# alipbcs/ZetaRay

Hardware: NVIDIA H100
Metric: Mpaths/s (1spp ReSTIR PT, 1080p) (higher is better)
Workload: dtype f32

## Files before the change

zetaray_b200/csrc/rpt.cu:

```cuda
#include "zr_rpt_io.cuh"
#include "zr_rpt_spatial.h"
#include "zr_schedule.h"

namespace zr
{
namespace
{
    using namespace RPT;

    __device__ __align__(8) float c_disk512[1024];

#ifndef ZR_PT_THREADS
#define ZR_PT_THREADS 768
#endif
    struct PtParked
    {
        Reservoir r;
        Reconnection rc;
        uint32_t pad;
    };
    static_assert(sizeof(PtParked) % 4 == 0 && (sizeof(PtParked) / 4) % 2 == 1, "PtParked must be an odd number of words");
    constexpr size_t PT_SMEM_BYTES = (size_t)ZR_PT_THREADS * sizeof(PtParked);

    template<uint32_t MF>
    __global__ void ZR_LB(ZR_PT_THREADS) k_pathtrace(SceneDev sc, FrameView f, RptParams prm, zr_rpt_reservoir* __restrict__ res,
        float4* __restrict__ target, float4* __restrict__ finalImg, uint32_t dispX, uint32_t dispY, const uint32_t* __restrict__ order)
    {
        using SD = BSDF::ShadingDataT<MF>;
        extern __shared__ PtParked s_ptParked[];
        const zr_frame_constants& fc = f.fc;
        const long long t0 = clock64();
        uint2 sg = make_uint2(0, 0);
        const uint32_t groupFlat = order[blockIdx.x] * (ZR_PT_THREADS / 128) + (threadIdx.x >> 7);
        const uint32_t tInGroup = threadIdx.x & 127;
        uint2 px = make_uint2(0xffffffffu, 0xffffffffu);
        if (groupFlat < dispX * dispY)
            px = SwizzleThreadGroup(groupFlat, 0, tInGroup & 15, tInGroup >> 4, 16, 8, dispX, 16, 4, 16 * dispY, sg);
        bool inBounds = px.x < f.W && px.y < f.H && px.y >= prm.rowBegin && px.y < prm.rowEnd;
        const size_t idx = (size_t)px.y * f.W + px.x;
        bool alive = false;
        if (inBounds)
        {
            const GFlags flags = FlagsAt(f.core, f.W, px.x, px.y);
            if (flags.invalid || flags.emissive)
            {
                if (!fc.Accumulate || !fc.CameraStatic)
                    finalImg[idx] = f4(0, 0, 0, 0);
                inBounds = false;
            }
        }
        float3 pos = f3(0), normal = f3(0), li = f3(0), throughput = f3(0), throughput_k = f3(1), tr = f3(1);
        SD surface;
        BSDF::BSDFSample bsdfSample = BSDF::BSDFSample::Init();
        HitEmissive nextHit;
        nextHit.hit = false;
        Reconnection& rc = s_ptParked[threadIdx.x].rc;
        Reservoir& r = s_ptParked[threadIdx.x].r;
        rc = Reconnection::Init();
        r = Reservoir::Init();
        PrevHit prevHit;
        prevHit.alpha_lobe = 0; prevHit.wi = f3(0); prevHit.pdf = 0; prevHit.lobe = BSDF::DIFFUSE_R;
        float eta_curr = BSDF::ETA_AIR, eta_next = BSDF::DEFAULT_ETA_MAT;
        bool inTranslucentMedium = false;
        int bounce = 0, maxNumBounces = 0;
        RNG rngReplay, rngThread, rngGroup;
        rngReplay.State = rngThread.State = rngGroup.State = 0;
        uint32_t sampleSetIdx = 0;
        uint32_t seedReplay0 = 0;

        if (inBounds)
        {
            const PixelT<SD> p = LoadPixel<SD>(f, sc, f.core, f.coat, px.x, px.y, false, px.x, px.y);
            rngGroup = RNG::Init4(sg.x, sg.y, fc.FrameNum, 1);
            const uint3 state = RNG::PCG3d(make_uint3(px.x, px.y, fc.FrameNum));
            rngReplay = RNG::InitSeed(state.x);
            rngThread = RNG::InitSeed(state.y);
            seedReplay0 = state.x;
            maxNumBounces = (int)(p.surface.specTr ? prm.maxGlossyTrBounces : prm.maxNonTrBounces);
            bsdfSample = BSDF::SampleBSDF(p.normal, p.surface, rngReplay);
            if (dot(bsdfSample.bsdfOverPdf, bsdfSample.bsdfOverPdf) != 0)
            {
                sampleSetIdx = rngGroup.UniformUintBounded_Faster(sc.numSampleSets);
                pos = p.pos; normal = p.normal; surface = p.surface;
                throughput = bsdfSample.bsdfOverPdf;
                prevHit.alpha_lobe = BSDF::LobeAlpha(p.surface, bsdfSample.lobe);
                prevHit.lobe = bsdfSample.lobe; prevHit.wi = bsdfSample.wi; prevHit.pdf = bsdfSample.pdf;
                eta_curr = dot(p.normal, bsdfSample.wi) < 0 ? p.eta_next : BSDF::ETA_AIR;
                inTranslucentMedium = eta_curr != BSDF::ETA_AIR;
                alive = true;
            }
        }
        ZR_PHASE();
        if (alive)
            nextHit = FindClosestEmissive(sc, pos, normal, bsdfSample.wi, surface.Transmissive());

        while (__syncthreads_or(alive))
        {
            bool atRR = false;
            Hit hitInfo;
            float prevBsdfSamplePdf = 0; BSDF::LOBE prevBsdfSampleLobe = BSDF::DIFFUSE_R;
            const int pathVertex = bounce + 2;
            if (alive && !nextHit.hit)
                alive = false;
            if (alive)
            {
                hitInfo = HitAttributes(sc, nextHit.geoIdx, nextHit.primIdx, nextHit.bary, nextHit.t);
                const float3 newPos = mad(hitInfo.t, bsdfSample.wi, pos);
                if (!GetMaterialData(sc, -bsdfSample.wi, eta_curr, hitInfo, surface, eta_next))
                    alive = false;
                else
                {
                    pos = newPos;
                    normal = hitInfo.normal;
                    prevBsdfSamplePdf = bsdfSample.pdf;
                    prevBsdfSampleLobe = bsdfSample.lobe;
                    tr = f3(1);
                    if (inTranslucentMedium && surface.TrDepthGt0())
                    {
                        const float3 c = surface.baseColor_Fr0_TrCol;
                        const float3 extCoeff = f3(-zr_logf(c.x), -zr_logf(c.y), -zr_logf(c.z)) / surface.trDepth;
                        tr = f3(zr_expf(-hitInfo.t * extCoeff.x), zr_expf(-hitInfo.t * extCoeff.y), zr_expf(-hitInfo.t * extCoeff.z));
                        throughput *= tr;
                    }
                }
            }
            ZR_PHASE();
            BSDF::BSDFSample nextBsdfSample = bsdfSample;
            const int nextBounce = pathVertex - 1;
            if (alive && nextBounce <= maxNumBounces)
                nextBsdfSample = BSDF::SampleBSDF(hitInfo.normal, surface, rngReplay);
            ZR_PHASE();
            RaySetup rs; rs.go = false;
            RayHit rh; rh.hit = false;
            if (alive)
            {
                rs = SetupClosestEmissive(pos, hitInfo.normal, nextBsdfSample.wi, surface.Transmissive());
                if (rs.go)
                    rh = TraceClosest(sc, rs.o, nextBsdfSample.wi, rs.tmin, FLT_MAX_);
            }
            ZR_PHASE();
            NeeLightState nee;
            nee.facing = false; nee.ld = f3(0);
            bool lightSample = false;
            uint32_t seed_nee = 0;
            if (alive)
            {
                nextHit = FinishClosestEmissive(sc, rs, rh, nextBsdfSample.wi);
                const DirectLightingEstimate ls_b = NEE_Bsdf_Finish(sc, pos, surface, nextBounce, maxNumBounces, nextBsdfSample, nextHit);
                if (nextHit.HitWasEmissive())
                {
                    const float3 fOverPdf = throughput * ls_b.ld;
                    li += fOverPdf;
                    rc.L = Reconnection::half3(ls_b.ld * throughput_k);
                    MaybeSetCase2OrCase3(pathVertex, pos, hitInfo.normal, hitInfo.t, hitInfo.ID, hitInfo.meshIdx, surface,
                        prevHit, ls_b, 0, rc, prm.alpha_min);
                    r.Update(Math::Luminance(fOverPdf), fOverPdf, rc, rngThread);
                }
                lightSample = !IsSpecularSurface(surface);
                if (lightSample)
                {
                    seed_nee = rngThread.State;
                    SD surfNee = surface;
                    nee = NEE_Emissive_Begin(sc, pos, hitInfo.normal, surfNee, sampleSetIdx, rngThread);
                }
            }
            ZR_PHASE();
            if (lightSample && nee.facing && dot(nee.ld, nee.ld) > 0)
            {
                const RaySetup seg = SetupSegment(pos, nee.ret.wi, nee.t, hitInfo.normal, nee.ret.ID, surface.Transmissive());
                const bool visible = seg.go ? !TraceAnyExcept(sc, seg.o, nee.ret.wi, seg.tmin, seg.tmax, nee.ret.ID) : false;
                nee.ld *= visible ? 1.0f : 0.0f;
            }
            ZR_PHASE();
            if (lightSample)
            {
                float bsdfPdf = 0;
                if (nee.facing && dot(nee.ld, nee.ld) > 0)
                {
                    SD surfNee = surface;
                    surfNee.SetWi(nee.ret.wi, hitInfo.normal);
                    bsdfPdf = BSDF::BSDFSamplerPdf(hitInfo.normal, surfNee, nee.ret.wi, rngThread);
                    bsdfPdf *= nee.dwdA;
                }
                const DirectLightingEstimate ls = NEE_Emissive_Finish(nee, bsdfPdf);
                const float3 fOverPdf = throughput * ls.ld;
                li += fOverPdf;
                if (rc.IsCase2() || rc.IsCase3())
                    rc.Clear();
                rc.L = Reconnection::half3(ls.ld * throughput_k);
                MaybeSetCase2OrCase3(pathVertex, pos, hitInfo.normal, hitInfo.t, hitInfo.ID, hitInfo.meshIdx, surface,
                    prevHit, ls, seed_nee, rc, prm.alpha_min);
                r.Update(Math::Luminance(fOverPdf), fOverPdf, rc, rngThread);
            }
            if (alive)
            {
                bsdfSample = nextBsdfSample;
                if (bounce >= (maxNumBounces - 1))
                    alive = false;
                else
                {
                    if (rc.IsCase2() || rc.IsCase3())
                        rc.Clear();
                    bounce++;
                    atRR = true;
                }
            }
            const uint32_t rrMask = __ballot_sync(0xffffffffu, atRR);
            if (rrMask == 0)
                continue;
            const int rrBounce = __shfl_sync(0xffffffffu, bounce, __ffs(rrMask) - 1);
            const bool doRR = prm.russianRoulette && (rrBounce >= 3);
            float waveThroughput = 0.0f;
            if (doRR)
                waveThroughput = WaveMax32(atRR ? Math::Luminance(throughput) : -FLT_MAX_);
            if (atRR)
            {
                do
                {
                    if (doRR && waveThroughput < 1)
                    {
                        const float p_terminate = fmaxf(0.05f, 1 - waveThroughput);
                        if (rngGroup.Uniform() < p_terminate) { alive = false; break; }
                        throughput /= (1 - p_terminate);
                        throughput_k /= ((int)rc.k <= bounce) ? (1 - p_terminate) : 1.0f;
                    }
                    if (dot(bsdfSample.bsdfOverPdf, bsdfSample.bsdfOverPdf) == 0) { alive = false; break; }
                    const float alpha_lobe = BSDF::LobeAlpha(surface, bsdfSample.lobe);
                    if (rc.Empty() && CanReconnect(prevHit.alpha_lobe, alpha_lobe, prevHit.lobe, bsdfSample.lobe, prm.alpha_min))
                    {
                        rc.SetCase1(pathVertex, pos, hitInfo.t, hitInfo.normal, hitInfo.ID, hitInfo.meshIdx, -surface.wo,
                            prevBsdfSampleLobe, prevBsdfSamplePdf, bsdfSample.wi, bsdfSample.lobe, bsdfSample.pdf);
                        throughput_k = f3(1);
                    }
                    if ((int)rc.k <= bounce)
                        throughput_k *= bsdfSample.bsdfOverPdf * tr;
                    const bool transmitted = dot(normal, bsdfSample.wi) < 0;
                    throughput *= bsdfSample.bsdfOverPdf;
                    eta_curr = transmitted ? (eta_curr == BSDF::ETA_AIR ? eta_next : BSDF::ETA_AIR) : eta_curr;
                    inTranslucentMedium = eta_curr != BSDF::ETA_AIR;
                    prevHit.alpha_lobe = alpha_lobe;
                    prevHit.lobe = bsdfSample.lobe;
                    prevHit.wi = bsdfSample.wi;
                    prevHit.pdf = bsdfSample.pdf;
                } while (false);
            }
        }

        AccountCost(prm.costMap, f.W, f.H, px.x, px.y, t0);
        if (!inBounds)
            return;
        r.rc.seed_replay = seedReplay0;
        const float targetLum = Math::Luminance(r.target);
        r.W = targetLum > 0 ? fmaxf(r.w_sum / targetLum, 1.0f) : 0;
        if (prm.temporalResample || prm.resetTemporal)
        {
            zr_rpt_reservoir rec;
            r.Write(rec, 0);
            StoreRecord(&res[idx], rec);
        }
        if (prm.temporalResample)
        {
            r.target = Math::Sanitize(r.target);
            target[idx] = f4(r.target.x, r.target.y, r.target.z, 0.0f);
        }
        else
        {
            li = isnan3(li) ? f3(0) : li;
            if (fc.Accumulate && fc.CameraStatic)
            {
                const float4 prev = finalImg[idx];
                finalImg[idx] = f4(prev.x + li.x, prev.y + li.y, prev.z + li.z, prev.w);
            }
            else
                finalImg[idx] = f4(li.x, li.y, li.z, 0.0f);
        }
    }

    __global__ void __launch_bounds__(256) k_spatial_search(FrameView f, RptParams prm, uint16_t* __restrict__ neighbor)
    {
        const zr_frame_constants& fc = f.fc;
        const uint32_t x = blockIdx.x * 32 + (threadIdx.x & 31);
        const uint32_t y = prm.rowBegin + blockIdx.y * 8 + (threadIdx.x >> 5);
        if (x >= f.W || y >= f.H || y >= prm.rowEnd) return;
        const size_t idx = (size_t)y * f.W + x;
        const uint4 c = ld128(&f.core[idx]);
        const GFlags flags = DecodeFlags(c.w & 0xff);
        if (flags.invalid || flags.emissive) return;
        const float roughness = (float)((c.w >> 8) & 0xff) / 255.0f;
        const float viewDepth = asfloat(c.x);
        const float2 renderDimF = f2((float)f.W, (float)f.H);
        const float2 jitter = f2(fc.CurrCameraJitter[0], fc.CurrCameraJitter[1]);
        const float3 pos = Math::WorldPosFromScreenSpace(f2((float)x, (float)y), renderDimF, viewDepth, fc.TanHalfFOV,
            fc.AspectRatio, fc.CurrViewInv, jitter);
        const float3 normal = Math::DecodeUnitVector(Math::DecodeUNorm2(c.y));
        const uint3 h = RNG::PCG3d(make_uint3(x, y, fc.FrameNum));
        RNG rng = RNG::Init(h.x, h.y, fc.FrameNum);
        const float u0 = rng.Uniform();
        const uint32_t offset = rng.UniformUint();
        const float theta = u0 * TWO_PI;
        float sinTheta, cosTheta;
        zr_sincosf(theta, &sinTheta, &cosTheta);
        int foundX = 0xffff, foundY = 0xffff;
        int sxs[3], sys[3];
        bool inside[3];
        uint4 cand[3];
#pragma unroll
        for (uint32_t i = 0; i < 3; i++)
        {
            const uint32_t si = (offset + i) & 511;
            const float2 sampleUV = __ldg(reinterpret_cast<const float2*>(c_disk512) + si);
            float2 rotated = f2(dot(sampleUV, f2(cosTheta, -sinTheta)), dot(sampleUV, f2(sinTheta, cosTheta)));
            rotated = rotated * 15.0f;
            sxs[i] = (int)rintf((float)x + rotated.x); sys[i] = (int)rintf((float)y + rotated.y);
            inside[i] = !(sxs[i] < 0 || sys[i] < 0 || sxs[i] >= (int)f.W || sys[i] >= (int)f.H) && !(sxs[i] == (int)x && sys[i] == (int)y);
            cand[i] = inside[i] ? ld128(&f.core[(size_t)sys[i] * f.W + sxs[i]]) : make_uint4(0, 0, 0, 0);
        }
#pragma unroll
        for (uint32_t i = 0; i < 3; i++)
        {
            if (foundX != 0xffff || !inside[i]) continue;
            const int sxp = sxs[i], syp = sys[i];
            const uint4 sc4 = cand[i];
            const GFlags sf = DecodeFlags(sc4.w & 0xff);
            if (sf.invalid || sf.emissive) continue;
            if (flags.metallic != sf.metallic) continue;
            if (flags.transmissive != sf.transmissive) continue;
            const float sampleRoughness = (float)((sc4.w >> 8) & 0xff) / 255.0f;
            if (fabsf(sampleRoughness - roughness) > 0.05f) continue;
            const float3 samplePos = Math::WorldPosFromScreenSpace(f2((float)sxp, (float)syp), renderDimF, asfloat(sc4.x),
                fc.TanHalfFOV, fc.AspectRatio, fc.CurrViewInv, jitter);
            const float3 sampleNormal = Math::DecodeUnitVector(Math::DecodeUNorm2(sc4.y));
            if (!(fabsf(dot(normal, samplePos - pos)) <= 0.01f * viewDepth)) continue;
            if (dot(sampleNormal, normal) < 0.9f) continue;
            foundX = sxp; foundY = syp;
        }
        uint32_t mx, my;
        if (foundX == 0xffff) { mx = 0xff; my = 0xff; }
        else { mx = (uint32_t)(foundX - (int)x + 32); my = (uint32_t)(foundY - (int)y + 32); }
        neighbor[idx] = (uint16_t)((mx & 0xff) | ((my & 0xff) << 8));
    }

    __global__ void __launch_bounds__(256) k_sort(FrameView f, int mode, uint32_t spatialFlag, const zr_rpt_reservoir* __restrict__ resCurr,
        const zr_rpt_reservoir* __restrict__ resPrev, const uint16_t* __restrict__ neighbor, uint16_t* __restrict__ threadMap,
        uint32_t dispX, uint32_t dispY, uint32_t tileRow0)
    {
        enum { SUCCESS = 0, INVALID_PIXEL = 1, NOT_FOUND = 2, EMPTY = 4 };
        __shared__ unsigned long long s_warp[8];
        const uint32_t Gx = blockIdx.x, Gy = blockIdx.y + tileRow0, Gidx = threadIdx.x;
        const uint32_t GTx = Gidx & 15, GTy = Gidx >> 4;
        const bool againstEdge = (Gx == dispX - 1) || (Gy == dispY - 1);
        const bool lastGroup = (Gx == dispX - 1) && (Gy == dispY - 1);
        int dxs[4], dys[4], cls[4];
        uint32_t result[4];
#pragma unroll
        for (int i = 0; i < 4; i++)
        {
            const int gtx = (int)GTx * 2 + (i & 1), gty = (int)GTy * 2 + (i >> 1);
            const int dx = (int)(Gx * 32) + gtx, dy = (int)(Gy * 32) + gty;
            dxs[i] = dx; dys[i] = dy;
            int nx = 0, ny = 0;
            uint32_t err = SUCCESS;
            if ((uint32_t)dx >= f.W || (uint32_t)dy >= f.H)
                err = INVALID_PIXEL;
            else
            {
                const GFlags flags = FlagsAt(f.core, f.W, dx, dy);
                if (flags.invalid || flags.emissive)
                    err = INVALID_PIXEL;
                else if (mode == 1)
                {
                    if (!PrevPixel(f, dx, dy, nx, ny)) err = NOT_FOUND;
                }
                else if (mode == 3)
                {
                    if (!NeighborOf(f, neighbor, dx, dy, nx, ny)) err = NOT_FOUND;
                }
            }
            bool skip = err != SUCCESS;
            uint32_t k = Reconnection::EMPTY;
            if (err == SUCCESS)
            {
                const zr_rpt_reservoir* src = (mode == 1) ? resPrev : resCurr;
                const int sx = (mode == 1 || mode == 3) ? nx : dx, sy = (mode == 1 || mode == 3) ? ny : dy;
                const uint32_t kk = __ldg(&src[(size_t)sy * f.W + sx].meta) & 0xf;
                k = kk == Reconnection::EMPTY ? kk : kk + 2;
            }
            uint32_t res = err;
            if (k == Reconnection::EMPTY) { res |= EMPTY; skip = true; }
            bool edge = false;
            if (skip && againstEdge && ((uint32_t)dx < f.W) && ((uint32_t)dy < f.H))
            {
                res = SUCCESS; skip = false; edge = true;
            }
            int c = 4;
            if (!skip)
            {
                if (k == 2) c = 0;
                else if (k == 3) c = 1;
                else if (k == 4) c = 2;
                else c = 3;
                (void)edge;
            }
            cls[i] = c;
            result[i] = res;
        }
        auto writeOutput = [&](int dx, int dy, int mgx, int mgy, uint32_t res)
        {
            if ((Gx == dispX - 1) && (Gy != dispY - 1)) { const int t = mgx; mgx = mgy; mgy = t; }
            const int mx = (int)(Gx * 32) + mgx, my = (int)(Gy * 32) + mgy;
            uint32_t error;
            if (mode == 1) error = res & (spatialFlag ? (INVALID_PIXEL | NOT_FOUND) : INVALID_PIXEL);
            else if (mode == 3) error = res & INVALID_PIXEL;
            else error = res & (INVALID_PIXEL | EMPTY);
            if ((uint32_t)mx < f.W && (uint32_t)my < f.H)
            {
                const uint32_t ux = (uint32_t)(dx - mx + 31), uy = (uint32_t)(dy - my + 31);
                threadMap[(size_t)my * f.W + mx] = (uint16_t)(ux | (uy << 7) | ((error > 0 ? 1u : 0u) << 15));
            }
        };
        if (lastGroup)
        {
#pragma unroll
            for (int i = 0; i < 4; i++)
                writeOutput(dxs[i], dys[i], (int)GTx * 2 + (i & 1), (int)GTy * 2 + (i >> 1), result[i]);
            return;
        }
        unsigned long long mine = 0;
#pragma unroll
        for (int i = 0; i < 4; i++) mine += 1ull << (11 * cls[i]);
        unsigned long long incl = mine;
        const uint32_t lane = Gidx & 31, warp = Gidx >> 5;
#pragma unroll
        for (int off = 1; off < 32; off <<= 1)
        {
            const unsigned long long n = __shfl_up_sync(0xffffffffu, incl, off);
            if (lane >= (uint32_t)off) incl += n;
        }
        if (lane == 31) s_warp[warp] = incl;
        __syncthreads();
        unsigned long long warpOff = 0, total = 0;
        for (uint32_t w = 0; w < 8; w++)
        {
            const unsigned long long v = s_warp[w];
            if (w < warp) warpOff += v;
            total += v;
        }
        const unsigned long long excl = warpOff + incl - mine;
        uint32_t base[5];
        uint32_t acc = 0;
#pragma unroll
        for (int c = 0; c < 5; c++) { base[c] = acc; acc += (uint32_t)((total >> (11 * c)) & 0x7ff); }
        uint32_t within[5] = { 0, 0, 0, 0, 0 };
#pragma unroll
        for (int i = 0; i < 4; i++)
        {
            const int c = cls[i];
            const uint32_t rank = base[c] + (uint32_t)((excl >> (11 * c)) & 0x7ff) + within[c];
            within[c]++;
            writeOutput(dxs[i], dys[i], (int)(rank & 31), (int)(rank >> 5), result[i]);
        }
    }
}
}

struct zr_indirect_pass
{
    uint32_t width = 0, height = 0;
    struct Sized
    {
        zr::Planes planes{ "zr_indirect_pass" };
        zr_rpt_reservoir* d_res[2] = { nullptr, nullptr };
        float4* d_target = nullptr;
        float4* d_final = nullptr;
        uint16_t* d_neighbor = nullptr;
        uint16_t* d_threadMap = nullptr;
        zr::SpatialQueued queued;
    } sz;
    zr::ShiftStreams shiftStreams;
    int currTemporalIdx = 0;
    bool isTemporalReservoirValid = false;
    bool resetTemporalTextures = true;
    bool patternLoaded = false;
    zr::LightingStrip strip{ "zr_indirect_pass" };
    zr_indirect_params params = Defaults();

    static zr_indirect_params Defaults()
    {
        zr_indirect_params p{};
        p.max_non_tr_bounces = 3; p.max_glossy_tr_bounces = 4; p.russian_roulette = 1; p.temporal_resample = 1;
        p.num_spatial_passes = 1; p.M_max_temporal = 10; p.M_max_spatial = 8; p.boiling_suppression = 1;
        p.sort_temporal = 1; p.sort_spatial = 1; p.alpha_min = 0.175f * 0.175f;
        return p;
    }

    zr_status Setup()
    {
        decltype(&zr::k_pathtrace<zr::BSDF::MF_ALL>) const kernels[2] = { zr::k_pathtrace<zr::BSDF::MF_NONE>, zr::k_pathtrace<zr::BSDF::MF_ALL> };
        for (const auto kernel : kernels)
            ZR_TRY(zr::ReserveParkedSmem(kernel, ZR_PT_THREADS, zr::PT_SMEM_BYTES, "zr_indirect_pass: k_pathtrace"));
        return shiftStreams.Init();
    }

    zr_status OnWindowResized(uint32_t w, uint32_t h)
    {
        const size_t n = (size_t)w * h;
        Sized next;
        for (int i = 0; i < 2; i++) ZR_TRY(next.planes.Alloc(next.d_res[i], n));
        ZR_TRY(next.planes.Alloc(next.d_threadMap, n));
        ZR_TRY(next.planes.Alloc(next.d_target, n));
        ZR_TRY(next.planes.Alloc(next.d_final, n));
        ZR_TRY(next.planes.Alloc(next.d_neighbor, n));
        ZR_TRY(next.queued.Build(w, h, next.d_res[0], next.d_res[1]));
        ZR_TRY(next.planes.Clear());
        sz = std::move(next);
        width = w; height = h;
        strip.ForgetSize();
        ResetFlags();
        return ZR_OK;
    }

    void ResetFlags() { currTemporalIdx = 0; isTemporalReservoirValid = false; resetTemporalTextures = true; }
    zr_status ResetTemporal()
    {
        ZR_TRY(sz.planes.Clear());
        ResetFlags();
        return ZR_OK;
    }

    zr_status LoadPattern()
    {
        if (patternLoaded) return ZR_OK;
        float pat[1024];
        zr_status st = zr::read_asset("zr_indirect_pass", "disk512.bin", pat, sizeof(pat));
        if (st != ZR_OK) return st;
        ZR_CUDA(cudaMemcpyToSymbol(zr::c_disk512, pat, 4096));
        patternLoaded = true;
        return ZR_OK;
    }

    zr_status Render(const zr_frame_inputs* in, cudaStream_t stream)
    {
        using namespace zr;
        FrameView f;
        zr_status st = LightingFrame("zr_indirect_pass", in, width, height, f);
        if (st != ZR_OK) return st;
        st = LoadPattern();
        if (st != ZR_OK) return st;

        const bool doTemporal = params.temporal_resample && isTemporalReservoirValid;
        const bool doSpatial = (params.num_spatial_passes > 0) && doTemporal;
        if (doTemporal && (!in->prev.d_core || !in->prev.d_coat))
        {
            set_error("zr_indirect_pass_render: temporal reuse needs the previous G-buffer");
            return ZR_ERR_INVALID_ARG;
        }
        RptParams prm;
        prm.maxNonTrBounces = params.max_non_tr_bounces; prm.maxGlossyTrBounces = params.max_glossy_tr_bounces;
        prm.russianRoulette = params.russian_roulette; prm.M_max_temporal = params.M_max_temporal; prm.M_max_spatial = params.M_max_spatial;
        prm.boilingSuppression = params.boiling_suppression; prm.sortSpatial = params.sort_spatial; prm.alpha_min = params.alpha_min;
        prm.temporalResample = doTemporal; prm.resetTemporal = resetTemporalTextures; prm.spatialFlag = doSpatial;
        prm.rowBegin = strip.rowBegin; prm.rowEnd = strip.ClampedRowEnd(height);
        prm.costMap = strip.d_costMap;
        st = strip.Schedule(width, height, 16, 8, ZR_PT_THREADS / 128);
        if (st != ZR_OK) return st;
        const uint32_t rows = prm.rowEnd - prm.rowBegin;

        int cur = currTemporalIdx;
        const uint32_t dispX = (width + 15) / 16, dispY = (height + 7) / 8;
        const bool plain = (in->scene->materialFeatures & BSDF::MF_ALL) == 0;
        ZR_PROF("k_pathtrace", stream);
        (plain ? k_pathtrace<BSDF::MF_NONE> : k_pathtrace<BSDF::MF_ALL>)<<<strip.sched[0].count, ZR_PT_THREADS, PT_SMEM_BYTES, stream>>>(in->scene->dev, f, prm, sz.d_res[cur], sz.d_target, sz.d_final, dispX, dispY,
            strip.sched[0].d_order);
        ZR_LAUNCH_CHECK();
        if (doTemporal)
        {
            st = sz.queued.RunTemporal(shiftStreams, in->scene->dev, f, prm, sz.d_res[cur], sz.d_res[1 - cur], sz.d_target, sz.d_final, plain, stream);
            if (st != ZR_OK) return st;
        }
        strip.Exchange(sz.d_res[cur], width, height, 64u, stream);
        if (doSpatial)
        {
            for (uint32_t pass = 0; pass < params.num_spatial_passes; pass++)
            {
                ZR_PROF("k_spatial_search", stream);
                k_spatial_search<<<dim3((width + 31) / 32, (rows + 7) / 8), 256, 0, stream>>>(f, prm, sz.d_neighbor);
                ZR_LAUNCH_CHECK();
                zr_rpt_reservoir* rin = sz.d_res[cur];
                zr_rpt_reservoir* rout = sz.d_res[1 - cur];
                cur = 1 - cur;
                if (params.sort_spatial)
                {
                    const uint32_t sx = (width + 31) / 32, sy = (height + 31) / 32;
                    ZR_PROF("k_sort", stream);
                    const uint32_t ty0 = prm.rowBegin / 32, ty1 = (prm.rowEnd + 31) / 32;
                    k_sort<<<dim3(sx, ty1 - ty0), 256, 0, stream>>>(f, 3, 1u, rin, nullptr, sz.d_neighbor, sz.d_threadMap, sx, sy, ty0);
                    ZR_LAUNCH_CHECK();
                }
                st = sz.queued.Run(shiftStreams, in->scene->dev, f, prm, rin, rout, sz.d_target, sz.d_final, sz.d_neighbor, sz.d_threadMap, plain, stream);
                if (st != ZR_OK) return st;
                strip.Exchange(rout, width, height, 64u, stream);
            }
        }
        isTemporalReservoirValid = true;
        currTemporalIdx = 1 - cur;
        resetTemporalTextures = false;
        return ZR_OK;
    }
};

extern "C"
{
    zr_status zr_indirect_pass_create(uint32_t width, uint32_t height, zr_indirect_pass** out) { return zr::CreatePass("zr_indirect_pass", width, height, out); }
    zr_status zr_indirect_pass_resize(zr_indirect_pass* p, uint32_t width, uint32_t height) { return zr::ResizePass("zr_indirect_pass", p, width, height); }
    zr_status zr_indirect_pass_reset_temporal(zr_indirect_pass* p) { return zr::ResetPass(p); }
    zr_status zr_indirect_pass_default_params(zr_indirect_params* out) { return zr::DefaultParams<zr_indirect_pass>(out); }
    zr_status zr_indirect_pass_set_params(zr_indirect_pass* p, const zr_indirect_params* params)
    {
        if (!p || !params) return ZR_ERR_INVALID_ARG;
        if (params->max_non_tr_bounces < 1 || params->max_non_tr_bounces > 8 || params->max_glossy_tr_bounces < 1 ||
            params->max_glossy_tr_bounces > 8 || params->M_max_temporal > 15 || params->M_max_spatial > 15 || params->num_spatial_passes > 2)
        {
            zr::set_error("zr_indirect_pass_set_params: value out of range (bounces 1..8, M_max <= 15, spatial passes <= 2)");
            return ZR_ERR_INVALID_ARG;
        }
        p->params = *params;
        return ZR_OK;
    }
    zr_status zr_indirect_pass_render(zr_indirect_pass* p, const zr_frame_inputs* in, void* stream)
    {
        if (!p) return ZR_ERR_INVALID_ARG;
        return p->Render(in, (cudaStream_t)stream);
    }
    zr_status zr_indirect_pass_get_output(zr_indirect_pass* p, zr_indirect_output id, zr_image2d* out)
    {
        if (!p || !out) return ZR_ERR_INVALID_ARG;
        const uint32_t w = p->width, h = p->height;
        switch (id)
        {
        case ZR_INDIRECT_FINAL: *out = zr_image2d{ p->sz.d_final, w, h, w * 16u, 16u }; break;
        case ZR_INDIRECT_RESERVOIR_CURR: *out = zr_image2d{ p->sz.d_res[1 - p->currTemporalIdx], w, h, w * 64u, 64u }; break;
        case ZR_INDIRECT_RESERVOIR_PREV: *out = zr_image2d{ p->sz.d_res[p->currTemporalIdx], w, h, w * 64u, 64u }; break;
        case ZR_INDIRECT_TARGET: *out = zr_image2d{ p->sz.d_target, w, h, w * 16u, 16u }; break;
        case ZR_INDIRECT_NEIGHBOR: *out = zr_image2d{ p->sz.d_neighbor, w, h, w * 2u, 2u }; break;
        case ZR_INDIRECT_THREADMAP_NTC: *out = zr_image2d{ p->sz.d_threadMap, w, h, w * 2u, 2u }; break;
        default: zr::set_error("zr_indirect_pass_get_output: unknown output id"); return ZR_ERR_INVALID_ARG;
        }
        return ZR_OK;
    }
    zr_status zr_indirect_pass_describe_io(zr_indirect_pass* p, zr_resource_use* uses, int* n)
    {
        if (!p || !uses || !n) return ZR_ERR_INVALID_ARG;
        uses[0] = zr_resource_use{ ZR_RES_GBUFFER_CURR, 0 };
        uses[1] = zr_resource_use{ ZR_RES_GBUFFER_PREV, 0 };
        uses[2] = zr_resource_use{ ZR_RES_SCENE_BVH, 0 };
        uses[3] = zr_resource_use{ ZR_RES_ALIAS_TABLE, 0 };
        uses[4] = zr_resource_use{ ZR_RES_INDIRECT_FINAL, 1 };
        *n = 5;
        return ZR_OK;
    }
    zr_status zr_indirect_pass_set_halo_exchange(zr_indirect_pass* p, zr_halo_exchange_fn fn, void* user) { return p ? p->strip.SetHaloExchange(fn, user) : ZR_ERR_INVALID_ARG; }
    zr_status zr_indirect_pass_set_schedule_costs(zr_indirect_pass* p, const double* h_tile_cost, uint32_t tiles_x, uint32_t tiles_y)
    {
        return p ? p->strip.SetScheduleCosts(h_tile_cost, tiles_x, tiles_y, p->width, p->height) : ZR_ERR_INVALID_ARG;
    }
    zr_status zr_indirect_pass_set_cost_map(zr_indirect_pass* p, void* d_cycles) { return p ? p->strip.SetCostMap(d_cycles) : ZR_ERR_INVALID_ARG; }
    zr_status zr_indirect_pass_set_rows(zr_indirect_pass* p, uint32_t y0, uint32_t y1) { return p ? p->strip.SetRows(y0, y1, p->height) : ZR_ERR_INVALID_ARG; }
    void zr_indirect_pass_destroy(zr_indirect_pass* p) { delete p; }
}
```

zetaray_b200/csrc/rpt_spatial.cu:

```cuda
#include "zr_rpt_spatial.h"
#include "zr_rpt_shift.cuh"
#include "zr_tma.cuh"

namespace zr
{
namespace
{
    using namespace RPT;

    __global__ void __launch_bounds__(256) k_spatial_classify(FrameView f, RptParams prm, const zr_rpt_reservoir* __restrict__ resIn,
        const uint16_t* __restrict__ neighbor, uint32_t* __restrict__ queue, uint32_t* __restrict__ counters, uint32_t capacity)
    {
        __shared__ uint32_t s_count[SpatialQueued::NUM_CLASSES], s_base[SpatialQueued::NUM_CLASSES];
        const uint32_t x = blockIdx.x * 32 + (threadIdx.x & 31);
        const uint32_t y = prm.rowBegin + blockIdx.y * 8 + (threadIdx.x >> 5);
        if (threadIdx.x < SpatialQueued::NUM_CLASSES) s_count[threadIdx.x] = 0;
        __syncthreads();
        uint32_t cls[2] = { NO_ITEM, NO_ITEM };
        if (x < f.W && y < f.H && y < prm.rowEnd)
        {
            const GFlags flags = FlagsAt(f.core, f.W, (int)x, (int)y);
            int nx = 0, ny = 0;
            if (!(flags.invalid || flags.emissive) && NeighborOf(f, neighbor, (int)x, (int)y, nx, ny))
            {
                const uint4 q0 = ld128(&resIn[(size_t)y * f.W + x]);
                const uint4 qn = ld128(&resIn[(size_t)ny * f.W + nx]);
                const bool selfEmpty = (q0.x & 0xf) == Reconnection::EMPTY, nEmpty = (qn.x & 0xf) == Reconnection::EMPTY;
                const uint32_t M_n = (qn.x >> 4) & 0xf;
                if (asfloat(q0.y) != 0 && !selfEmpty && M_n > 0) cls[0] = ShiftClass(q0.x);
                if (!nEmpty) cls[1] = ShiftClass(qn.x);
            }
        }
        const uint32_t item[2] = { x | (y << 16), x | (y << 16) | (1u << 31) };
        AppendItems(cls, item, queue, counters, capacity, s_count, s_base);
    }

    struct MergeSmem
    {
        uint4 rec[2][1024][4];
        float val[2][1024];
        float sum[2][1024];
        uint8_t cls[1024];
        uint8_t visited[1024];
        unsigned long long bar[2];
    };

    __global__ void __launch_bounds__(1024, 1) k_spatial_merge(const CUtensorMap* __restrict__ pMapIn, FrameView f, RptParams prm,
        const zr_rpt_reservoir* __restrict__ resIn, zr_rpt_reservoir* __restrict__ resOut, const float4* __restrict__ target,
        float4* __restrict__ finalImg, const uint16_t* __restrict__ neighbor, const uint16_t* __restrict__ threadMap,
        const ShiftResult* __restrict__ shiftRes, uint32_t tilesX, uint32_t tileRow0, uint32_t numTiles, uint32_t swizzled)
    {
        extern __shared__ __align__(1024) unsigned char smemRaw[];
        MergeSmem& sm = *reinterpret_cast<MergeSmem*>(smemRaw);
        const zr_frame_constants& fc = f.fc;
        const uint32_t t = threadIdx.x, lane = t & 31, warp = t >> 5;
        constexpr uint32_t TILE_BYTES = 1024 * 64;

        if (t == 0)
        {
            tma::MbarInit(reinterpret_cast<uint64_t*>(&sm.bar[0]), 1);
            tma::MbarInit(reinterpret_cast<uint64_t*>(&sm.bar[1]), 1);
            tma::FenceBarrierInit();
        }
        __syncthreads();
        auto issue = [&](uint32_t tile, uint32_t stage)
        {
            const uint32_t tx = tile % tilesX, ty = tileRow0 + tile / tilesX;
            uint64_t* bar = reinterpret_cast<uint64_t*>(&sm.bar[stage]);
            tma::MbarArriveExpectTx(bar, TILE_BYTES);
            if (swizzled) tma::Load3D(&sm.rec[stage][0][0], pMapIn, bar, 0, (int32_t)(tx * 16), (int32_t)(ty * 32));
            else tma::Load2D(&sm.rec[stage][0][0], pMapIn, bar, (int32_t)(tx * 32 * 8), (int32_t)(ty * 32));
        };
        if (t == 0 && blockIdx.x < numTiles)
            issue(blockIdx.x, 0);

        uint32_t pfFlags = 0xff, pfNb = 0xffff, pfMap = 0x8000;
        float4 pfTg = f4(0, 0, 0, 0);
        auto prefetch = [&](uint32_t tile)
        {
            const uint32_t tX = tile % tilesX, tY = tileRow0 + tile / tilesX;
            const uint32_t px = tX * 32 + lane, py = tY * 32 + warp;
            pfFlags = 0xff; pfNb = 0xffff; pfMap = 0x8000;
            if (px < f.W && py < f.H && py >= prm.rowBegin && py < prm.rowEnd)
            {
                const size_t i = (size_t)py * f.W + px;
                pfFlags = __ldg(&f.core[i].w) & 0xff;
                pfNb = __ldg(&neighbor[i]);
                pfTg = __ldg(&target[i]);
            }
            const uint32_t sx = tX * 32 + (warp & 3) * 8 + (lane & 7), sy = tY * 32 + (warp >> 2) * 4 + (lane >> 3);
            if (sx < f.W && sy < f.H)
                pfMap = prm.sortSpatial ? __ldg(&threadMap[(size_t)sy * f.W + sx]) : (31u | (31u << 7));
        };
        if (blockIdx.x < numTiles)
            prefetch(blockIdx.x);

        uint32_t it = 0;
        for (uint32_t tile = blockIdx.x; tile < numTiles; tile += gridDim.x, it++)
        {
            const uint32_t stage = it & 1, parity = (it >> 1) & 1;
            const uint32_t tileX = tile % tilesX, tileY = tileRow0 + tile / tilesX;
            if (t == 0 && tile + gridDim.x < numTiles)
            {
                tma::FenceProxyAsync();
                issue(tile + gridDim.x, stage ^ 1);
            }
            const int x = (int)(tileX * 32 + lane), y = (int)(tileY * 32 + warp);
            const bool inImage = (uint32_t)x < f.W && (uint32_t)y < f.H;
            const size_t idx = inImage ? (size_t)y * f.W + x : 0;
            bool act = false;
            {
                const GFlags flags = DecodeFlags(pfFlags);
                act = !(flags.invalid || flags.emissive);
            }
            int nx = 0, ny = 0;
            bool hasN = false;
            const float4 tg = pfTg;
            const uint32_t mapEnc = pfMap;
            uint4 sh0 = make_uint4(0, 0, 0, 0);
            float2 sh1 = f2(0, 0);
            uint4 n0 = make_uint4(Reconnection::EMPTY, 0, 0, 0), n1 = make_uint4(0, 0, 0, 0);
            if (act)
            {
                const uint32_t ox = pfNb & 0xff, oy = pfNb >> 8;
                hasN = ox != 0xff;
                nx = (int)ox - 32 + x; ny = (int)oy - 32 + y;
                if (hasN)
                {
                    const uint4* nrec = reinterpret_cast<const uint4*>(&resIn[(size_t)ny * f.W + nx]);
                    n0 = __ldg(&nrec[0]); n1 = __ldg(&nrec[1]);
                    asm volatile("prefetch.global.L1 [%0];" :: "l"(nrec + 2));
                    const uint4* sp = reinterpret_cast<const uint4*>(&shiftRes[idx]);
                    sh0 = __ldg(&sp[0]);
                    sh1 = __ldg(reinterpret_cast<const float2*>(&sp[1]));
                }
            }
            if (tile + gridDim.x < numTiles)
                prefetch(tile + gridDim.x);
            sm.visited[t] = 0;
            tma::MbarWait(reinterpret_cast<uint64_t*>(&sm.bar[stage]), parity);

            zr_rpt_reservoir rec;
            {
                const uint4* line = &sm.rec[stage][t & ~1u][0];
                const uint32_t c0 = (t & 1u) * 4u, sw = swizzled ? ((t >> 1) & 7u) : 0u;
                uint4 v[4] = { line[(c0 + 0) ^ sw], line[(c0 + 1) ^ sw], line[(c0 + 2) ^ sw], line[(c0 + 3) ^ sw] };
                memcpy(&rec, v, 64);
            }
            Reservoir r_curr = Reservoir::Load_NonReconnection(rec);
            r_curr.target = f3(tg.x, tg.y, tg.z);
            const float wsum0 = act ? r_curr.w_sum : 0.0f;
            uint32_t M_max = prm.M_max_spatial;
            M_max = !r_curr.rc.Empty() && r_curr.rc.lobe_k_min_1 == BSDF::GLOSSY_T ? (M_max < 4 ? M_max : 4) : M_max;
            uint32_t cls = 0, M_new = 0;
            bool changed = false, surfKMin1Tr = false;
            zr_rpt_reservoir recN;
            Reservoir r_spatial = Reservoir::Init();
            if (act && !hasN)
                cls = 1;
            else if (act)
            {
                memset(&recN, 0, sizeof(recN));
                memcpy(&recN, &n0, 16); memcpy(reinterpret_cast<unsigned char*>(&recN) + 16, &n1, 16);
                r_spatial = Reservoir::Load_NonReconnection(recN);
                if ((r_curr.w_sum != 0) && !r_curr.rc.Empty() && (r_spatial.M > 0))
                {
                    const float target_spatial = sh1.x;
                    if (target_spatial > 0)
                    {
                        const float selfJ = (r_curr.rc.IsCase3() && r_curr.rc.lobe_k_min_1 == BSDF::ALL) ? 1.0f : asfloat(rec.jacobian_or_seed_nee);
                        const float targetLum_curr = r_curr.W > 0 ? r_curr.w_sum / r_curr.W : 0;
                        const float jacobian = selfJ > 0 ? sh1.y / selfJ : 0;
                        const float numerator = (float)r_curr.M * targetLum_curr;
                        const float denom = numerator + (float)r_spatial.M * target_spatial * jacobian;
                        const float m_curr = denom > 0 ? numerator / denom : 0;
                        r_curr.w_sum *= m_curr;
                    }
                }
                M_new = r_curr.M + r_spatial.M;
                if (r_spatial.rc.Empty())
                    cls = 2;
                else
                {
                    cls = 3;
                    M_max = r_spatial.rc.x_k_in_motion ? (M_max < 4 ? M_max : 4) : M_max;
                    r_spatial.rc.x_k_in_motion = false;
                    const float nJ = (r_spatial.rc.IsCase3() && r_spatial.rc.lobe_k_min_1 == BSDF::ALL) ? 1.0f : asfloat(recN.jacobian_or_seed_nee);
                    const float3 shTarget = f3(asfloat(sh0.x), asfloat(sh0.y), asfloat(sh0.z));
                    const float shJ = fabsf(asfloat(sh0.w));
                    surfKMin1Tr = (sh0.w >> 31) != 0;
                    const float targetLum_curr = Math::Luminance(shTarget);
                    const float targetLum_spatial = r_spatial.W > 0 ? r_spatial.w_sum / r_spatial.W : 0;
                    const float jacobian = nJ > 0 ? shJ / nJ : 0;
                    if (targetLum_curr > 1e-6f && jacobian > 1e-5f && jacobian < 100)
                    {
                        const uint3 h = RNG::PCG3d(make_uint3((uint32_t)x, (uint32_t)y, (uint32_t)y));
                        RNG rng = RNG::Init(h.x, h.z, fc.FrameNum + 511);
                        const float numerator = (float)r_spatial.M * targetLum_spatial;
                        const float denom = numerator / jacobian + (float)r_curr.M * targetLum_curr;
                        const float m_spatial = denom > 0 ? numerator / denom : 0;
                        const float w_spatial = m_spatial * r_spatial.W * targetLum_curr;
                        if (r_curr.Update(w_spatial, shTarget, r_spatial.rc, rng))
                        {
                            const uint4* nrec = reinterpret_cast<const uint4*>(&resIn[(size_t)ny * f.W + nx]);
                            const uint4 n2 = __ldg(&nrec[2]), n3 = __ldg(&nrec[3]);
                            memcpy(reinterpret_cast<unsigned char*>(&recN) + 32, &n2, 16);
                            memcpy(reinterpret_cast<unsigned char*>(&recN) + 48, &n3, 16);
                            r_spatial.Load_Reconnection(recN);
                            r_curr.rc = r_spatial.rc;
                            r_curr.rc.partialJacobian = shJ;
                            changed = true;
                        }
                    }
                    const float targetLum = Math::Luminance(r_curr.target);
                    r_curr.W = targetLum > 0 ? r_curr.w_sum / targetLum : 0;
                    r_curr.M = M_new;
                }
            }
            sm.val[0][t] = wsum0;
            sm.val[1][t] = act ? r_curr.w_sum : 0.0f;
            sm.cls[t] = (uint8_t)cls;
            __syncthreads();

            {
                const int sx = (int)(tileX * 32 + (warp & 3) * 8 + (lane & 7)), sy = (int)(tileY * 32 + (warp >> 2) * 4 + (lane >> 3));
                bool on = (uint32_t)sx < f.W && (uint32_t)sy < f.H;
                int lx = sx - (int)(tileX * 32), ly = sy - (int)(tileY * 32);
                if (mapEnc & (1u << 15)) on = false;
                lx += (int)(mapEnc & 0x3f) - 31;
                ly += (int)((mapEnc >> 7) & 0x3f) - 31;
                if (on && ((uint32_t)lx >= 32u || (uint32_t)ly >= 32u)) on = false;
                const uint32_t lp = on ? (uint32_t)(ly * 32 + lx) : 0;
                const float v0 = on ? sm.val[0][lp] : 0.0f, v1 = on ? sm.val[1][lp] : 0.0f;
                const uint32_t c = on ? sm.cls[lp] : 0;
                const float waveSum = WaveSum32(v0);
                float waveAcc = WaveSum32(c == 1 ? v1 : 0.0f);
                waveAcc += WaveSum32(c == 2 ? v1 : 0.0f);
                const float total = waveAcc + WaveSum32(c == 3 ? v1 : 0.0f);
                if (on)
                {
                    sm.sum[0][lp] = waveSum; sm.sum[1][lp] = total;
                    sm.visited[lp] = 1;
                }
            }
            __syncthreads();

            if (act && sm.visited[t])
            {
                const float avgEx0 = (sm.sum[0][t] - wsum0) / 32.0f;
                if (cls == 1)
                {
                    if (prm.boilingSuppression) SuppressOutlier(avgEx0, r_curr);
                    WriteOutputColor(fc, finalImg, idx, r_curr.target * r_curr.W);
                    CopyToNextFrame(rec, &resOut[idx], r_curr, M_max);
                }
                else if (cls == 2)
                {
                    if (prm.boilingSuppression) SuppressOutlier(avgEx0, r_curr);
                    const float targetLum = Math::Luminance(r_curr.target);
                    r_curr.W = targetLum > 0 ? r_curr.w_sum / targetLum : 0;
                    r_curr.M = M_new;
                    CopyToNextFrame(rec, &resOut[idx], r_curr, M_max);
                    WriteOutputColor(fc, finalImg, idx, r_curr.target * r_curr.W);
                }
                else
                {
                    if (prm.boilingSuppression)
                        SuppressOutlier((sm.sum[1][t] - r_curr.w_sum) / 32.0f, r_curr);
                    if (changed)
                    {
                        const uint32_t mmax = surfKMin1Tr ? (M_max < 4 ? M_max : 4) : M_max;
                        zr_rpt_reservoir out;
                        r_curr.Write(out, mmax);
                        StoreRecord(&resOut[idx], out);
                    }
                    else
                        CopyToNextFrame(rec, &resOut[idx], r_curr, M_max);
                    WriteOutputColor(fc, finalImg, idx, r_curr.target * r_curr.W);
                }
            }
            __syncthreads();
        }
    }
}

zr_status ShiftStreams::Init()
{
    int dev = 0;
    ZR_CUDA(cudaGetDevice(&dev));
    ZR_CUDA(cudaDeviceGetAttribute(&numSMs, cudaDevAttrMultiProcessorCount, dev));
    ZR_CUDA(cudaFuncSetAttribute(k_spatial_merge, cudaFuncAttributeMaxDynamicSharedMemorySize, (int)sizeof(MergeSmem)));
    ZR_TRY(SetupShifts<false>());
    ZR_TRY(SetupTemporalShifts());
    for (int i = 0; i < 2; i++)
    {
        ZR_CUDA(cudaStreamCreateWithFlags(&aux[i], cudaStreamNonBlocking));
        ZR_CUDA(cudaEventCreateWithFlags(&evJoin[i], cudaEventDisableTiming));
    }
    ZR_CUDA(cudaEventCreateWithFlags(&evFork, cudaEventDisableTiming));
    return ZR_OK;
}

ShiftStreams::~ShiftStreams()
{
    for (int i = 0; i < 2; i++)
    {
        if (aux[i]) cudaStreamDestroy(aux[i]);
        if (evJoin[i]) cudaEventDestroy(evJoin[i]);
    }
    if (evFork) cudaEventDestroy(evFork);
}

zr_status SpatialQueued::Build(uint32_t w, uint32_t h, const zr_rpt_reservoir* res0, const zr_rpt_reservoir* res1)
{
    width = w; height = h;
    const size_t n = (size_t)w * h;
    capacity = 2 * n;
    ZR_TRY(planes.Alloc(d_queue, NUM_CLASSES * capacity, false));
    ZR_TRY(planes.Alloc(d_counters, 16, false));
    ZR_TRY(planes.Alloc(d_shift, n));
    ZR_TRY(planes.Alloc(d_flags, n));
    ZR_TRY(planes.Alloc(d_maps, 2, false));
    const zr_rpt_reservoir* res[2] = { res0, res1 };
    CUtensorMap maps[2];
    swizzled = (w % 2) == 0;
    for (int i = 0; i < 2; i++)
    {
        mapBase[i] = res[i];
        bool ok;
        if (swizzled)
        {
            const uint64_t dims[3] = { 16, w / 2, h };
            const uint64_t strides[2] = { 128, (uint64_t)w * 64 };
            const uint32_t box[3] = { 16, 16, 32 };
            ok = tma::EncodeWords(&maps[i], res[i], 3, dims, strides, box, true);
        }
        else
            ok = tma::EncodePlane2D(&maps[i], res[i], w, h, 64, (uint64_t)w * 64, 32, 32);
        if (!ok)
        {
            set_error("zr_indirect_pass: cuTensorMapEncodeTiled failed for the %ux%u reservoir plane", w, h);
            return ZR_ERR_CUDA;
        }
    }
    ZR_CUDA(cudaMemcpy(d_maps, maps, sizeof(maps), cudaMemcpyHostToDevice));
    return planes.Clear();
}

zr_status SpatialQueued::Run(const ShiftStreams& ss, const SceneDev& sc, const FrameView& f, const RptParams& prm, const zr_rpt_reservoir* resIn,
    zr_rpt_reservoir* resOut, const float4* target, float4* finalImg, const uint16_t* neighbor, const uint16_t* threadMap, bool plain, cudaStream_t stream)
{
    const int plane = resIn == mapBase[0] ? 0 : (resIn == mapBase[1] ? 1 : -1);
    if (plane < 0) { set_error("zr_indirect_pass: spatial input is not one of the pass's reservoir planes"); return ZR_ERR_INVALID_ARG; }
    const uint32_t rows = prm.rowEnd - prm.rowBegin;
    ZR_CUDA(cudaMemsetAsync(d_counters, 0, 16 * sizeof(uint32_t), stream));
    {
        ZR_PROF("k_spatial_classify", stream);
        k_spatial_classify<<<dim3((width + 31) / 32, (rows + 7) / 8), 256, 0, stream>>>(f, prm, resIn, neighbor, d_queue, d_counters, (uint32_t)capacity);
        ZR_LAUNCH_CHECK();
    }
    {
        ZR_PROF("k_shift", stream);
        const zr_status ls = LaunchShifts<false>(*this, ss, sc, f, prm, resIn, nullptr, neighbor, plain, stream);
        zr::prof_after();
        if (ls != ZR_OK) return ls;
        cudaError_t e = cudaGetLastError();
        if (e != cudaSuccess) return zr::cuda_fail(e, "k_shift launch");
    }
    {
        const uint32_t tilesX = (width + 31) / 32;
        const uint32_t tileRow0 = prm.rowBegin / 32, tileRow1 = (prm.rowEnd + 31) / 32;
        const uint32_t numTiles = tilesX * (tileRow1 - tileRow0);
        const uint32_t grid = numTiles < (uint32_t)ss.numSMs ? numTiles : (uint32_t)ss.numSMs;
        ZR_PROF("k_spatial_merge", stream);
        k_spatial_merge<<<grid, 1024, sizeof(MergeSmem), stream>>>(d_maps + plane, f, prm, resIn, resOut, target, finalImg, neighbor, threadMap,
            d_shift, tilesX, tileRow0, numTiles, swizzled ? 1u : 0u);
        ZR_LAUNCH_CHECK();
    }
    return ZR_OK;
}
}
```

zetaray_b200/csrc/rpt_temporal.cu:

```cuda
#include "zr_rpt_spatial.h"
#include "zr_rpt_shift.cuh"

namespace zr
{
namespace
{
    using namespace RPT;
    enum : uint8_t { TF_OK = 1, TF_REPLAY_OK = 2 };

    __global__ void __launch_bounds__(256) k_temporal_classify(SceneDev sc, FrameView f, RptParams prm, const zr_rpt_reservoir* __restrict__ resCurr,
        const zr_rpt_reservoir* __restrict__ resPrev, uint8_t* __restrict__ tflags, uint32_t* __restrict__ queue, uint32_t* __restrict__ counters,
        uint32_t capacity)
    {
        __shared__ uint32_t s_count[SpatialQueued::NUM_CLASSES], s_base[SpatialQueued::NUM_CLASSES];
        const int x = (int)(blockIdx.x * 32 + (threadIdx.x & 31));
        const int y = (int)(prm.rowBegin + blockIdx.y * 8 + (threadIdx.x >> 5));
        if (threadIdx.x < SpatialQueued::NUM_CLASSES) s_count[threadIdx.x] = 0;
        __syncthreads();
        uint32_t cls[2] = { NO_ITEM, NO_ITEM };
        uint32_t flagBits = 0;
        if (x < (int)f.W && y < (int)f.H && y < (int)prm.rowEnd)
        {
            const size_t idx = (size_t)y * f.W + x;
            const GFlags flags = DecodeFlags(ld128(&f.core[idx]).w & 0xff);
            bool ok = !(flags.invalid || flags.emissive), okReplay = false;
            int ppx = 0, ppy = 0;
            if (ok)
            {
                ok = PrevPixel(f, x, y, ppx, ppy);
                if (ok)
                    ok = asfloat(__ldg(&f.pcore[(size_t)ppy * f.W + ppx].x)) != FLT_MAX_;
            }
            if (ok)
            {
                const Pixel cur = LoadPixel(f, sc, f.core, f.coat, x, y, false, x, y);
                const Pixel prev = LoadPixel(f, sc, f.pcore, f.pcoat, ppx, ppy, true, x, y);
                ok = PlaneHeuristic(prev.pos, cur.normal, cur.pos, cur.z, 1.0f);
                okReplay = ok && PlaneHeuristic(prev.pos, cur.normal, cur.pos, cur.z, 0.01f);
                const bool matOk = !(prev.flags.emissive || (fabsf(prev.roughness - cur.roughness) > 0.3f) ||
                    (prev.flags.transmissive != cur.flags.transmissive));
                ok = ok && matOk;
                okReplay = okReplay && matOk;
            }
            if (ok)
            {
                flagBits = TF_OK | (okReplay ? TF_REPLAY_OK : 0);
                const uint4 q0 = ld128(&resCurr[idx]);
                const uint4 qp = ld128(&resPrev[(size_t)ppy * f.W + ppx]);
                const bool selfEmpty = (q0.x & 0xf) == Reconnection::EMPTY, pEmpty = (qp.x & 0xf) == Reconnection::EMPTY;
                const uint32_t M_p = (qp.x >> 4) & 0xf;
                if (asfloat(q0.y) != 0 && M_p > 0 && !selfEmpty) cls[0] = ShiftClass(q0.x);
                if (!pEmpty) cls[1] = ShiftClass(qp.x);
            }
            tflags[idx] = (uint8_t)flagBits;
        }
        const uint32_t base = (uint32_t)x | ((uint32_t)y << 16) | ((flagBits & TF_REPLAY_OK) ? (1u << 30) : 0u);
        const uint32_t item[2] = { base, base | (1u << 31) };
        AppendItems(cls, item, queue, counters, capacity, s_count, s_base);
    }

    __global__ void __launch_bounds__(256, 4) k_temporal_merge(SceneDev sc, FrameView f, RptParams prm, zr_rpt_reservoir* __restrict__ resCurr,
        const zr_rpt_reservoir* __restrict__ resPrev, float4* __restrict__ target, float4* __restrict__ finalImg,
        const uint8_t* __restrict__ tflags, const ShiftResult* __restrict__ shiftRes)
    {
        const zr_frame_constants& fc = f.fc;
        const int x = (int)(blockIdx.x * 32 + (threadIdx.x & 31));
        const int y = (int)(prm.rowBegin + blockIdx.y * 8 + (threadIdx.x >> 5));
        if (x >= (int)f.W || y >= (int)f.H || y >= (int)prm.rowEnd) return;
        const size_t idx = (size_t)y * f.W + x;
        {
            const GFlags flags = DecodeFlags(ld128(&f.core[idx]).w & 0xff);
            if (flags.invalid || flags.emissive) return;
        }
        zr_rpt_reservoir rec;
        LoadRecord(&resCurr[idx], rec);
        Reservoir r_curr = Reservoir::Load_NonReconnection(rec);
        const float4 tg = target[idx];
        r_curr.target = f3(tg.x, tg.y, tg.z);
        const bool ok = (__ldg(&tflags[idx]) & TF_OK) != 0;
        if (!ok)
        {
            if (!prm.spatialFlag)
                WriteOutputColor(fc, finalImg, idx, r_curr.target * r_curr.W);
            return;
        }
        int ppx = 0, ppy = 0;
        PrevPixel(f, x, y, ppx, ppy);
        const size_t pidx = (size_t)ppy * f.W + ppx;
        zr_rpt_reservoir recPrev;
        LoadRecord(&resPrev[pidx], recPrev);
        Reservoir r_prev = Reservoir::Load_NonReconnection(recPrev);
        const uint4* sp = reinterpret_cast<const uint4*>(&shiftRes[idx]);

        if (r_curr.w_sum != 0 && r_prev.M > 0 && !r_curr.rc.Empty())
        {
            const float2 sh1 = __ldg(reinterpret_cast<const float2*>(&sp[1]));
            const float target_prev = sh1.x;
            if (target_prev > 0)
            {
                const float selfJ = (r_curr.rc.IsCase3() && r_curr.rc.lobe_k_min_1 == BSDF::ALL) ? 1.0f : asfloat(rec.jacobian_or_seed_nee);
                const float targetLum_curr = r_curr.W > 0 ? r_curr.w_sum / r_curr.W : 0;
                const float jacobian = selfJ > 0 ? sh1.y / selfJ : 0;
                const float m_curr = targetLum_curr / (targetLum_curr + (float)r_prev.M * target_prev * jacobian);
                r_curr.w_sum *= m_curr;
                rec.w_sum = r_curr.w_sum;
            }
        }

        const uint32_t M_new = r_curr.M + r_prev.M;
        const uint32_t M_max = prm.M_max_temporal;
        if (r_prev.rc.Empty())
        {
            const float targetLum = Math::Luminance(r_curr.target);
            r_curr.W = targetLum > 0 ? r_curr.w_sum / targetLum : 0;
            r_curr.M = M_new;
            const uint32_t k = r_curr.rc.Empty() ? r_curr.rc.k : (r_curr.rc.k > 2 ? r_curr.rc.k : 2) - 2;
            const uint32_t mm = r_curr.M < M_max ? r_curr.M : M_max;
            rec.meta = (rec.meta & 0xffffff00u) | ((k | (mm << 4)) & 0xff);
            rec.W = r_curr.W;
            st128(&resCurr[idx], make_uint4(rec.meta, asuint(rec.w_sum), asuint(rec.W), rec.L_b));
            if (!prm.spatialFlag)
                WriteOutputColor(fc, finalImg, idx, r_curr.target * r_curr.W);
            return;
        }
        r_prev.Load_Reconnection(recPrev);
        if (r_prev.rc.IsCase1() || r_prev.rc.IsCase2())
            XkToCurr(sc, r_prev.rc);
        const uint4 sh0 = __ldg(&sp[0]);
        const float3 shTarget = f3(asfloat(sh0.x), asfloat(sh0.y), asfloat(sh0.z));
        const float shJ = asfloat(sh0.w);
        const float targetLum_curr = Math::Luminance(shTarget);
        const float jacobian = r_prev.rc.partialJacobian > 0 ? shJ / r_prev.rc.partialJacobian : 0;
        bool changed = false;
        if (targetLum_curr > 1e-6f && jacobian > 1e-5f)
        {
            RNG rng = RNG::Init((uint32_t)y, (uint32_t)x, fc.FrameNum + 31);
            const float targetLum_prev = r_prev.W > 0 ? r_prev.w_sum / r_prev.W : 0;
            const float numerator = (float)r_prev.M * targetLum_prev;
            const float denom = numerator / jacobian + targetLum_curr;
            const float m_prev = denom > 0 ? numerator / denom : 0;
            const float w_prev = m_prev * r_prev.W * targetLum_curr;
            if (r_curr.Update(w_prev, shTarget, r_prev.rc, rng))
            {
                r_curr.rc.partialJacobian = shJ;
                changed = true;
            }
        }
        const float targetLum = Math::Luminance(r_curr.target);
        r_curr.W = targetLum > 0 ? r_curr.w_sum / targetLum : 0;
        r_curr.M = M_new;
        if (changed)
        {
            zr_rpt_reservoir out;
            r_curr.Write(out, M_max);
            StoreRecord(&resCurr[idx], out);
            if (prm.spatialFlag)
            {
                r_curr.target = Math::Sanitize(r_curr.target);
                target[idx] = f4(r_curr.target.x, r_curr.target.y, r_curr.target.z, 0.0f);
            }
        }
        else
        {
            r_curr.WriteReservoirData(rec, M_max);
            st128(&resCurr[idx], make_uint4(rec.meta, asuint(rec.w_sum), asuint(rec.W), rec.L_b));
        }
        if (!prm.spatialFlag)
            WriteOutputColor(fc, finalImg, idx, r_curr.target * r_curr.W);
    }
}

zr_status SetupTemporalShifts()
{
    return SetupShifts<true>();
}

zr_status SpatialQueued::RunTemporal(const ShiftStreams& ss, const SceneDev& sc, const FrameView& f, const RptParams& prm, zr_rpt_reservoir* resCurr,
    const zr_rpt_reservoir* resPrev, float4* target, float4* finalImg, bool plain, cudaStream_t stream)
{
    const uint32_t rows = prm.rowEnd - prm.rowBegin;
    const dim3 grid((width + 31) / 32, (rows + 7) / 8);
    ZR_CUDA(cudaMemsetAsync(d_counters, 0, 16 * sizeof(uint32_t), stream));
    {
        ZR_PROF("k_temporal_classify", stream);
        k_temporal_classify<<<grid, 256, 0, stream>>>(sc, f, prm, resCurr, resPrev, d_flags, d_queue, d_counters, (uint32_t)capacity);
        ZR_LAUNCH_CHECK();
    }
    {
        ZR_PROF("k_shift_temporal", stream);
        const zr_status ls = LaunchShifts<true>(*this, ss, sc, f, prm, resCurr, resPrev, nullptr, plain, stream);
        zr::prof_after();
        if (ls != ZR_OK) return ls;
        cudaError_t e = cudaGetLastError();
        if (e != cudaSuccess) return zr::cuda_fail(e, "k_shift (temporal) launch");
    }
    {
        ZR_PROF("k_temporal_merge", stream);
        k_temporal_merge<<<grid, 256, 0, stream>>>(sc, f, prm, resCurr, resPrev, target, finalImg, d_flags, d_shift);
        ZR_LAUNCH_CHECK();
    }
    return ZR_OK;
}
}
```

zetaray_b200/csrc/zr_rpt_io.cuh:

```cuda
#pragma once
#include "zr_rpt.cuh"
#include "zr_pixel.cuh"

namespace zr
{
struct RptParams
{
    uint32_t maxNonTrBounces, maxGlossyTrBounces, russianRoulette, M_max_temporal, M_max_spatial;
    uint32_t boilingSuppression, sortSpatial;
    float alpha_min;
    uint32_t temporalResample, resetTemporal, spatialFlag;
    uint32_t rowBegin, rowEnd;
    unsigned long long* costMap;
};

namespace
{
    using namespace RPT;

    ZR_D void LoadRecord(const zr_rpt_reservoir* __restrict__ p, zr_rpt_reservoir& r)
    {
        const uint4* q = reinterpret_cast<const uint4*>(p);
        uint4 v[4] = { q[0], q[1], q[2], q[3] };
        memcpy(&r, v, 64);
    }
    ZR_D void StoreRecord(zr_rpt_reservoir* __restrict__ p, const zr_rpt_reservoir& r)
    {
        uint4 v[4];
        memcpy(v, &r, 64);
        uint4* q = reinterpret_cast<uint4*>(p);
        q[0] = v[0]; q[1] = v[1]; q[2] = v[2]; q[3] = v[3];
    }
    ZR_D uint4 LoadQ0(const zr_rpt_reservoir* __restrict__ p) { return *reinterpret_cast<const uint4*>(p); }

    ZR_D bool NeighborOf(const FrameView& f, const uint16_t* __restrict__ neighbor, int x, int y, int& nx, int& ny)
    {
        const uint16_t nb = __ldg(&neighbor[(size_t)y * f.W + x]);
        const int ox = nb & 0xff, oy = nb >> 8;
        if (ox == 0xff) return false;
        nx = ox - 32 + x; ny = oy - 32 + y;
        return true;
    }

    ZR_D void SuppressOutlier(float waveAvgExclusive, Reservoir& r)
    {
        if (r.w_sum > 50 * waveAvgExclusive)
        {
            r.M = 0; r.w_sum = 0; r.W = 0; r.rc.Clear();
        }
    }

    ZR_D bool RecordSurvivesRoundTrip(const zr_rpt_reservoir& in)
    {
        const uint32_t wx = in.w_k & 0xffff, wy = in.w_k >> 16;
        const bool interior = wx != 0 && wx != 0xffff && wy != 0 && wy != 0xffff;
        const uint32_t r = in.L_rg & 0x7fff, g = (in.L_rg >> 16) & 0x7fff, b = in.L_b & 0x7fff;
        return interior && r <= 0x7c00 && g <= 0x7c00 && b <= 0x7c00;
    }

    ZR_D void CopyToNextFrame(const zr_rpt_reservoir& in, zr_rpt_reservoir* __restrict__ outPtr, Reservoir r_curr, uint32_t M_max)
    {
        if (!r_curr.rc.Empty() && RecordSurvivesRoundTrip(in))
        {
            zr_rpt_reservoir out = in;
            out.meta = r_curr.PackMeta(M_max);
            out.w_sum = Math::Sanitize(r_curr.w_sum);
            out.W = Math::Sanitize(r_curr.W);
            out.L_b = in.L_b & 0xffff;
            if (r_curr.rc.IsCase1()) { out.lightPdf = 0; out.dwdA = 0; out.seed_nee = 0; }
            else if (!r_curr.rc.IsCase2()) { out.dwdA = 0; out.seed_nee = 0; out.meshIdx = 0; }
            StoreRecord(outPtr, out);
        }
        else if (!r_curr.rc.Empty())
        {
            r_curr.Load_Reconnection(in);
            zr_rpt_reservoir out;
            r_curr.Write(out, M_max);
            StoreRecord(outPtr, out);
        }
        else
        {
            const uint4 old = LoadQ0(outPtr);
            const uint32_t k = r_curr.rc.k;
            const uint32_t mm = r_curr.M < M_max ? r_curr.M : M_max;
            st128(outPtr, make_uint4((old.x & 0xffffff00u) | ((k | (mm << 4)) & 0xff), asuint(r_curr.w_sum), asuint(r_curr.W), old.w));
        }
    }

    ZR_D bool PrevPixel(const FrameView& f, int x, int y, int& ppx, int& ppy)
    {
        const float2 renderDim = f2((float)f.W, (float)f.H);
        const float2 motionVec = unpack_snorm16x2(__ldg(&f.me[(size_t)y * f.W + x].x));
        const float2 currUV = f2((float)x + 0.5f, (float)y + 0.5f) / renderDim;
        const float2 prevUV = currUV - motionVec;
        const float2 pp = prevUV * renderDim;
        ppx = (int)pp.x; ppy = (int)pp.y;
        return !(prevUV.x < 0.0f || prevUV.y < 0.0f || prevUV.x > 1.0f || prevUV.y > 1.0f);
    }

    ZR_D bool PlaneHeuristic(float3 prevPos, float3 normal, float3 pos, float linearDepth, float th)
    {
        return fabsf(dot(normal, prevPos - pos)) <= th * linearDepth;
    }

    ZR_D void XkToPrev(const SceneDev& sc, Reconnection& rc)
    {
        const zr_mesh_instance md = LoadInstance(sc, rc.meshIdx);
        const float4 q_curr = normalize(Math::DecodeNormalized4(md.Rotation));
        const float3 T = f3(md.Translation[0], md.Translation[1], md.Translation[2]);
        const float3 x_local = Math::InverseTransformTRS(rc.x_k, T, q_curr, h3(md.Scale));
        const float3 prevTranslation = T - h3(md.dTranslation);
        const float4 q_prev = normalize(Math::DecodeNormalized4(md.PrevRotation));
        rc.x_k = Math::TransformTRS(x_local, prevTranslation, q_prev, h3(md.PrevScale));
    }
    ZR_D void XkToCurr(const SceneDev& sc, Reconnection& rc)
    {
        const zr_mesh_instance md = LoadInstance(sc, rc.meshIdx);
        const float3 T = f3(md.Translation[0], md.Translation[1], md.Translation[2]);
        const float3 dT = h3(md.dTranslation);
        const float3 prevTranslation = T - dT;
        const float4 q_prev = normalize(Math::DecodeNormalized4(md.PrevRotation));
        const float3 prevScale = h3(md.PrevScale), scale = h3(md.Scale);
        const float3 x_local = Math::InverseTransformTRS(rc.x_k, prevTranslation, q_prev, prevScale);
        const float4 q_curr = normalize(Math::DecodeNormalized4(md.Rotation));
        rc.x_k = Math::TransformTRS(x_local, T, q_curr, scale);
        const float4 dRot = f4(q_prev.x - q_curr.x, q_prev.y - q_curr.y, q_prev.z - q_curr.z, q_prev.w - q_curr.w);
        const float3 dScale = prevScale - scale;
        rc.x_k_in_motion = dot(dT, dT) > 0;
        rc.x_k_in_motion = rc.x_k_in_motion || dot(dRot, dRot) > 0;
        rc.x_k_in_motion = rc.x_k_in_motion || dot(dScale, dScale) > 0;
    }

    struct PrevHit { float alpha_lobe; float3 wi; float pdf; BSDF::LOBE lobe; };

    template<class SD>
    ZR_D void MaybeSetCase2OrCase3(int pathVertex, float3 pos, float3 normal, float t, uint32_t ID, uint32_t meshIdx,
        const SD& surface, const PrevHit& prevHit, const DirectLightingEstimate& ls, uint32_t seed_nee,
        Reconnection& rc, float alpha_min)
    {
        const float alpha_lobe_direct = BSDF::LobeAlpha(surface, ls.lobe);
        if (rc.Empty() && CanReconnect(prevHit.alpha_lobe, alpha_lobe_direct, prevHit.lobe, ls.lobe, alpha_min))
        {
            rc.SetCase2(pathVertex, pos, t, normal, ID, meshIdx, prevHit.wi, prevHit.lobe, prevHit.pdf, ls.wi, ls.lobe,
                ls.pdf_solidAngle, ls.lt, ls.pdf_light, ls.le, seed_nee, ls.dwdA);
        }
        if (rc.Empty() && (alpha_lobe_direct >= alpha_min))
        {
            rc.SetCase3(pathVertex + 1, ls.pos, ls.lt, ls.lobe, ls.ID, ls.le, ls.normal, ls.pdf_solidAngle, ls.pdf_light,
                ls.dwdA, ls.wi, ls.twoSided, seed_nee);
        }
    }

}
}
```

zetaray_b200/csrc/zr_rpt_shift.cuh:

```cuda
#pragma once
#include "zr_rpt_spatial.h"

namespace zr
{
namespace
{
    using namespace RPT;
#ifndef ZR_SHIFT_THREADS
#define ZR_SHIFT_THREADS 768
#endif
#ifndef ZR_SHIFT_MINBLOCKS
#define ZR_SHIFT_MINBLOCKS 1
#endif
    constexpr int SHIFT_THREADS = ZR_SHIFT_THREADS, SHIFT_MINBLOCKS = ZR_SHIFT_MINBLOCKS;
    constexpr uint32_t NO_ITEM = 0xffffffffu;

    struct ShiftParked
    {
        Reconnection rc;
        uint32_t pad;
    };
    static_assert(sizeof(ShiftParked) % 4 == 0 && (sizeof(ShiftParked) / 4) % 2 == 1, "ShiftParked must be an odd number of words");
    constexpr size_t SHIFT_SMEM_BYTES = (size_t)SHIFT_THREADS * sizeof(ShiftParked);

    ZR_D uint32_t ShiftClass(uint32_t meta)
    {
        const uint32_t kMin2 = meta & 0xf;
        const uint32_t lt_k = (meta >> 14) & 3, lt_k1 = (meta >> 16) & 3;
        const uint32_t c = lt_k1 != 0 ? 1u : (lt_k != 0 ? 2u : 0u);
        return c * 2 + (kMin2 > 0 ? 1u : 0u);
    }


    template<int CASE, bool REPLAY, bool TEMPORAL, uint32_t MF>
    __global__ void __launch_bounds__(SHIFT_THREADS, SHIFT_MINBLOCKS) k_shift(SceneDev sc, FrameView f, RptParams prm,
        const zr_rpt_reservoir* __restrict__ resIn, const zr_rpt_reservoir* __restrict__ resPrev, const uint16_t* __restrict__ neighbor,
        const uint32_t* __restrict__ queue, uint32_t* __restrict__ counters, uint32_t cls, ShiftResult* __restrict__ out)
    {
        using SD = BSDF::ShadingDataT<MF>;
        __shared__ uint32_t s_base;
        extern __shared__ ShiftParked s_shiftParked[];
        Reconnection& rc = s_shiftParked[threadIdx.x].rc;
        const uint32_t total = counters[cls];
        for (;;)
        {
            __syncthreads();
            if (threadIdx.x == 0) s_base = atomicAdd(&counters[8 + cls], (uint32_t)SHIFT_THREADS);
            __syncthreads();
            const uint32_t base = s_base;
            if (base >= total) break;
            const bool act = base + threadIdx.x < total;
            int x = 0, y = 0;
            uint32_t dir = 0;
            bool replayOk = act;
            PixelT<SD> p, pr;
            if (act)
            {
                const uint32_t item = __ldg(&queue[base + threadIdx.x]);
                x = (int)(item & 0xffff); y = (int)((item >> 16) & 0x3fff); dir = item >> 31;
                zr_rpt_reservoir rec;
                if (!TEMPORAL)
                {
                    int nx = 0, ny = 0;
                    NeighborOf(f, neighbor, x, y, nx, ny);
                    LoadRecord(dir == 0 ? &resIn[(size_t)y * f.W + x] : &resIn[(size_t)ny * f.W + nx], rec);
                    Reservoir r = Reservoir::Load_NonReconnection(rec);
                    r.rc.x_k_in_motion = false;
                    r.Load_Reconnection(rec);
                    rc = r.rc;
                    if (dir == 0) p = LoadPixel<SD>(f, sc, f.core, f.coat, nx, ny, false, x, y);
                    else p = LoadPixel<SD>(f, sc, f.core, f.coat, x, y, false, x, y);
                    if (REPLAY)
                    {
                        if (dir == 0) pr = LoadPixel<SD>(f, sc, f.core, f.coat, nx, ny, false, nx, ny);
                        else pr = p;
                    }
                }
                else
                {
                    replayOk = ((item >> 30) & 1) != 0;
                    int ppx = 0, ppy = 0;
                    PrevPixel(f, x, y, ppx, ppy);
                    LoadRecord(dir == 0 ? &resIn[(size_t)y * f.W + x] : &resPrev[(size_t)ppy * f.W + ppx], rec);
                    Reservoir r = Reservoir::Load_NonReconnection(rec);
                    r.Load_Reconnection(rec);
                    if (r.rc.IsCase1() || r.rc.IsCase2())
                    {
                        if (dir == 0) XkToPrev(sc, r.rc);
                        else XkToCurr(sc, r.rc);
                    }
                    rc = r.rc;
                    if (dir == 0) p = LoadPixel<SD>(f, sc, f.pcore, f.pcoat, ppx, ppy, true, x, y);
                    else p = LoadPixel<SD>(f, sc, f.core, f.coat, x, y, false, x, y);
                    if (REPLAY) pr = p;
                }
            }
            else
                rc = Reconnection::Init();
            OffsetPathContextT<SD> ctx = OffsetPathContextT<SD>::Init();
            if (REPLAY)
            {
                ZR_PHASE();
                ctx = Replay_kGt2_Sync(act && replayOk, sc, pr.pos, pr.normal, pr.eta_next, pr.surface, rc, prm.alpha_min);
                if (act && replayOk)
                    ctx = ctx.Quantize();
            }
            const OffsetPath shift = Shift2_Sync<CASE>(act, sc, p.pos, p.normal, p.eta_next, p.surface, rc, &ctx, prm.alpha_min);
            if (act)
            {
                ShiftResult* o = &out[(size_t)y * f.W + x];
                if (dir == 0)
                    *reinterpret_cast<float2*>(&o->ctsTargetLum) = f2(Math::Luminance(shift.target), shift.partialJacobian);
                else if (TEMPORAL)
                    st128(o, make_uint4(asuint(shift.target.x), asuint(shift.target.y), asuint(shift.target.z), asuint(shift.partialJacobian)));
                else
                {
                    const float J = shift.partialJacobian;
                    const float Jenc = J > 0 ? (shift.surfKMin1Tramsmissive ? -J : J) : 0.0f;
                    st128(o, make_uint4(asuint(shift.target.x), asuint(shift.target.y), asuint(shift.target.z), asuint(Jenc)));
                }
            }
        }
    }

    template<bool TEMPORAL>
    zr_status LaunchShifts(const SpatialQueued& q, const ShiftStreams& ss, const SceneDev& sc, const FrameView& f, const RptParams& prm,
        const zr_rpt_reservoir* resIn, const zr_rpt_reservoir* resPrev, const uint16_t* neighbor, bool plain, cudaStream_t stream)
    {
        const uint32_t grid = (uint32_t)ss.numSMs * SHIFT_MINBLOCKS;
        cudaStream_t s1 = ss.aux[0], s2 = ss.aux[1];
        ZR_CUDA(cudaEventRecord(ss.evFork, stream));
        ZR_CUDA(cudaStreamWaitEvent(s1, ss.evFork, 0));
        ZR_CUDA(cudaStreamWaitEvent(s2, ss.evFork, 0));
#define ZR_LAUNCH_SHIFT(CASE, REPLAY, CLS, STREAM) \
        (plain ? k_shift<CASE, REPLAY, TEMPORAL, BSDF::MF_NONE> : k_shift<CASE, REPLAY, TEMPORAL, BSDF::MF_ALL>)<<<grid, SHIFT_THREADS, SHIFT_SMEM_BYTES, STREAM>>>(sc, f, prm, resIn, resPrev, neighbor, q.d_queue + (size_t)(CLS) * q.capacity, \
            q.d_counters, CLS, q.d_shift); \
        zr::count_launch()
        ZR_LAUNCH_SHIFT(1, false, 0, stream);
        ZR_LAUNCH_SHIFT(2, false, 2, s1);
        ZR_LAUNCH_SHIFT(3, false, 4, s2);
        ZR_LAUNCH_SHIFT(1, true, 1, s1);
        ZR_LAUNCH_SHIFT(2, true, 3, s2);
        ZR_LAUNCH_SHIFT(3, true, 5, stream);
#undef ZR_LAUNCH_SHIFT
        ZR_CUDA(cudaEventRecord(ss.evJoin[0], s1));
        ZR_CUDA(cudaEventRecord(ss.evJoin[1], s2));
        ZR_CUDA(cudaStreamWaitEvent(stream, ss.evJoin[0], 0));
        ZR_CUDA(cudaStreamWaitEvent(stream, ss.evJoin[1], 0));
        return ZR_OK;
    }

    template<bool TEMPORAL>
    zr_status SetupShifts()
    {
        using BSDF::MF_NONE; using BSDF::MF_ALL;
        decltype(&k_shift<1, false, TEMPORAL, MF_ALL>) const kernels[12] = {
            k_shift<1, false, TEMPORAL, MF_NONE>, k_shift<2, false, TEMPORAL, MF_NONE>, k_shift<3, false, TEMPORAL, MF_NONE>,
            k_shift<1, true, TEMPORAL, MF_NONE>, k_shift<2, true, TEMPORAL, MF_NONE>, k_shift<3, true, TEMPORAL, MF_NONE>,
            k_shift<1, false, TEMPORAL, MF_ALL>, k_shift<2, false, TEMPORAL, MF_ALL>, k_shift<3, false, TEMPORAL, MF_ALL>,
            k_shift<1, true, TEMPORAL, MF_ALL>, k_shift<2, true, TEMPORAL, MF_ALL>, k_shift<3, true, TEMPORAL, MF_ALL> };
        for (const auto kernel : kernels)
            ZR_TRY(ReserveParkedSmem(kernel, SHIFT_THREADS, SHIFT_SMEM_BYTES, "zr_indirect_pass: k_shift"));
        return ZR_OK;
    }

    ZR_D void AppendItems(const uint32_t cls[2], const uint32_t item[2], uint32_t* __restrict__ queue, uint32_t* __restrict__ counters,
        uint32_t capacity, uint32_t* s_count, uint32_t* s_base)
    {
        const uint32_t lane = threadIdx.x & 31;
        uint32_t offs[2] = { 0, 0 };
        const uint32_t lt = (1u << lane) - 1;
#pragma unroll
        for (uint32_t c = 0; c < SpatialQueued::NUM_CLASSES; c++)
        {
            const uint32_t m0 = __ballot_sync(0xffffffffu, cls[0] == c), m1 = __ballot_sync(0xffffffffu, cls[1] == c);
            const uint32_t n0 = __popc(m0), n = n0 + __popc(m1);
            uint32_t base = 0;
            if (n && lane == 0) base = atomicAdd(&s_count[c], n);
            base = __shfl_sync(0xffffffffu, base, 0);
            if (cls[0] == c) offs[0] = base + __popc(m0 & lt);
            if (cls[1] == c) offs[1] = base + n0 + __popc(m1 & lt);
        }
        __syncthreads();
        if (threadIdx.x < SpatialQueued::NUM_CLASSES)
            s_base[threadIdx.x] = s_count[threadIdx.x] ? atomicAdd(&counters[threadIdx.x], s_count[threadIdx.x]) : 0;
        __syncthreads();
#pragma unroll
        for (uint32_t d = 0; d < 2; d++)
            if (cls[d] != NO_ITEM)
                queue[(size_t)cls[d] * capacity + s_base[cls[d]] + offs[d]] = item[d];
    }
}
}
```

zetaray_b200/csrc/zr_rpt_spatial.h:

```cpp
#pragma once
#include <cuda.h>
#include "zr_planes.h"
#include "zr_rpt_io.cuh"

namespace zr
{
struct ShiftResult
{
    float stcTarget[3];
    float stcJacobian;
    float ctsTargetLum;
    float ctsJacobian;
    uint32_t pad[2];
};
static_assert(sizeof(ShiftResult) == 32, "ShiftResult is two 128-bit words");

struct ShiftStreams
{
    int numSMs = 0;
    cudaStream_t aux[2] = { nullptr, nullptr };
    cudaEvent_t evFork = nullptr, evJoin[2] = { nullptr, nullptr };
    ShiftStreams() = default;
    ShiftStreams(const ShiftStreams&) = delete;
    ShiftStreams& operator=(const ShiftStreams&) = delete;
    ~ShiftStreams();
    zr_status Init();
};
zr_status SetupTemporalShifts();

struct SpatialQueued
{
    static constexpr int NUM_CLASSES = 6;
    Planes planes{ "zr_indirect_pass" };
    uint32_t width = 0, height = 0;
    uint32_t* d_queue = nullptr;
    uint32_t* d_counters = nullptr;
    ShiftResult* d_shift = nullptr;
    uint8_t* d_flags = nullptr;
    size_t capacity = 0;
    const void* mapBase[2] = { nullptr, nullptr };
    CUtensorMap* d_maps = nullptr;
    bool swizzled = false;

    zr_status Build(uint32_t w, uint32_t h, const zr_rpt_reservoir* res0, const zr_rpt_reservoir* res1);
    zr_status Run(const ShiftStreams& ss, const SceneDev& sc, const FrameView& f, const RptParams& prm, const zr_rpt_reservoir* resIn,
        zr_rpt_reservoir* resOut, const float4* target, float4* finalImg, const uint16_t* neighbor, const uint16_t* threadMap, bool plain,
        cudaStream_t stream);
    zr_status RunTemporal(const ShiftStreams& ss, const SceneDev& sc, const FrameView& f, const RptParams& prm, zr_rpt_reservoir* resCurr,
        const zr_rpt_reservoir* resPrev, float4* target, float4* finalImg, bool plain, cudaStream_t stream);
};
}
```

zetaray_b200/csrc/zr_tma.cuh:

```cuda
#pragma once
#include <cuda.h>
#include <cuda_runtime.h>
#include <cstdint>

namespace zr
{
namespace tma
{
    inline bool EncodePlane2D(CUtensorMap* map, const void* base, uint32_t width, uint32_t height, uint32_t recordBytes,
        uint64_t pitchBytes, uint32_t boxW, uint32_t boxH)
    {
        typedef CUresult (*EncodeFn)(CUtensorMap*, CUtensorMapDataType, cuuint32_t, void*, const cuuint64_t*, const cuuint64_t*,
            const cuuint32_t*, const cuuint32_t*, CUtensorMapInterleave, CUtensorMapSwizzle, CUtensorMapL2promotion, CUtensorMapFloatOOBfill);
        static EncodeFn encode = nullptr;
        if (!encode)
        {
            void* fn = nullptr;
            cudaDriverEntryPointQueryResult qres;
            if (cudaGetDriverEntryPoint("cuTensorMapEncodeTiled", &fn, cudaEnableDefault, &qres) != cudaSuccess || !fn ||
                qres != cudaDriverEntryPointSuccess)
                return false;
            encode = (EncodeFn)fn;
        }
        const uint32_t wordsPerRecord = recordBytes / 8;
        if (recordBytes % 8 || pitchBytes % 16 || boxW * wordsPerRecord > 256 || boxH > 256 || ((uintptr_t)base & 15))
            return false;
        const cuuint64_t dims[2] = { (cuuint64_t)width * wordsPerRecord, height };
        const cuuint64_t strides[1] = { pitchBytes };
        const cuuint32_t box[2] = { boxW * wordsPerRecord, boxH };
        const cuuint32_t elemStrides[2] = { 1, 1 };
        return encode(map, CU_TENSOR_MAP_DATA_TYPE_UINT64, 2, const_cast<void*>(base), dims, strides, box, elemStrides,
            CU_TENSOR_MAP_INTERLEAVE_NONE, CU_TENSOR_MAP_SWIZZLE_NONE, CU_TENSOR_MAP_L2_PROMOTION_L2_128B,
            CU_TENSOR_MAP_FLOAT_OOB_FILL_NONE) == CUDA_SUCCESS;
    }

    inline bool EncodeWords(CUtensorMap* map, const void* base, uint32_t rank, const uint64_t* dims, const uint64_t* stridesBytes, const uint32_t* box,
        bool swizzle128 = false)
    {
        typedef CUresult (*EncodeFn)(CUtensorMap*, CUtensorMapDataType, cuuint32_t, void*, const cuuint64_t*, const cuuint64_t*,
            const cuuint32_t*, const cuuint32_t*, CUtensorMapInterleave, CUtensorMapSwizzle, CUtensorMapL2promotion, CUtensorMapFloatOOBfill);
        static EncodeFn encode = nullptr;
        if (!encode)
        {
            void* fn = nullptr;
            cudaDriverEntryPointQueryResult qres;
            if (cudaGetDriverEntryPoint("cuTensorMapEncodeTiled", &fn, cudaEnableDefault, &qres) != cudaSuccess || !fn ||
                qres != cudaDriverEntryPointSuccess)
                return false;
            encode = (EncodeFn)fn;
        }
        if (rank < 1 || rank > 5 || ((uintptr_t)base & 15) || (box[0] * 8) % 16) return false;
        cuuint64_t d[5]; cuuint64_t st[4]; cuuint32_t b[5]; cuuint32_t es[5];
        for (uint32_t i = 0; i < rank; i++) { d[i] = dims[i]; b[i] = box[i]; es[i] = 1; if (box[i] == 0 || box[i] > 256) return false; }
        for (uint32_t i = 0; i + 1 < rank; i++) { st[i] = stridesBytes[i]; if (st[i] % 16) return false; }
        if (swizzle128 && box[0] != 16) return false;
        return encode(map, CU_TENSOR_MAP_DATA_TYPE_UINT64, rank, const_cast<void*>(base), d, st, b, es,
            CU_TENSOR_MAP_INTERLEAVE_NONE, swizzle128 ? CU_TENSOR_MAP_SWIZZLE_128B : CU_TENSOR_MAP_SWIZZLE_NONE, CU_TENSOR_MAP_L2_PROMOTION_L2_128B,
            CU_TENSOR_MAP_FLOAT_OOB_FILL_NONE) == CUDA_SUCCESS;
    }

#ifdef __CUDACC__
    __device__ __forceinline__ uint32_t SmemAddr(const void* p) { return (uint32_t)__cvta_generic_to_shared(p); }

    __device__ __forceinline__ void MbarInit(uint64_t* bar, uint32_t arrivals)
    {
        asm volatile("mbarrier.init.shared::cta.b64 [%1], %0;" :: "r"(arrivals), "r"(SmemAddr(bar)) : "memory");
    }
    __device__ __forceinline__ void FenceBarrierInit() { asm volatile("fence.mbarrier_init.release.cluster;" ::: "memory"); }
    __device__ __forceinline__ void FenceProxyAsync() { asm volatile("fence.proxy.async.shared::cta;" ::: "memory"); }

    __device__ __forceinline__ void MbarArriveExpectTx(uint64_t* bar, uint32_t bytes)
    {
        asm volatile("mbarrier.arrive.expect_tx.shared::cta.b64 _, [%1], %0;" :: "r"(bytes), "r"(SmemAddr(bar)) : "memory");
    }
    __device__ __forceinline__ void MbarWait(uint64_t* bar, uint32_t parity)
    {
        asm volatile(
            "{\n\t"
            ".reg .pred P1;\n\t"
            "LAB_WAIT:\n\t"
            "mbarrier.try_wait.parity.shared::cta.b64 P1, [%0], %1, %2;\n\t"
            "@P1 bra DONE;\n\t"
            "bra LAB_WAIT;\n\t"
            "DONE:\n\t"
            "}" :: "r"(SmemAddr(bar)), "r"(parity), "r"(0x989680u) : "memory");
    }
    __device__ __forceinline__ void Load2D(void* smem, const CUtensorMap* map, uint64_t* bar, int32_t x0, int32_t y0)
    {
        asm volatile("cp.async.bulk.tensor.2d.shared::cluster.global.mbarrier::complete_tx::bytes [%0], [%1, {%3, %4}], [%2];"
            :: "r"(SmemAddr(smem)), "l"((uint64_t)map), "r"(SmemAddr(bar)), "r"(x0), "r"(y0) : "memory");
    }
    __device__ __forceinline__ void Store2D(const CUtensorMap* map, const void* smem, int32_t x0, int32_t y0)
    {
        asm volatile("cp.async.bulk.tensor.2d.global.shared::cta.bulk_group [%0, {%2, %3}], [%1];"
            :: "l"((uint64_t)map), "r"(SmemAddr(smem)), "r"(x0), "r"(y0) : "memory");
    }
    __device__ __forceinline__ void Load3D(void* smem, const CUtensorMap* map, uint64_t* bar, int32_t c0, int32_t c1, int32_t c2)
    {
        asm volatile("cp.async.bulk.tensor.3d.shared::cluster.global.mbarrier::complete_tx::bytes [%0], [%1, {%3, %4, %5}], [%2];"
            :: "r"(SmemAddr(smem)), "l"((uint64_t)map), "r"(SmemAddr(bar)), "r"(c0), "r"(c1), "r"(c2) : "memory");
    }
    __device__ __forceinline__ void Load4D(void* smem, const CUtensorMap* map, uint64_t* bar, int32_t c0, int32_t c1, int32_t c2, int32_t c3)
    {
        asm volatile("cp.async.bulk.tensor.4d.shared::cluster.global.mbarrier::complete_tx::bytes [%0], [%1, {%3, %4, %5, %6}], [%2];"
            :: "r"(SmemAddr(smem)), "l"((uint64_t)map), "r"(SmemAddr(bar)), "r"(c0), "r"(c1), "r"(c2), "r"(c3) : "memory");
    }
    __device__ __forceinline__ void Store4D(const CUtensorMap* map, const void* smem, int32_t c0, int32_t c1, int32_t c2, int32_t c3)
    {
        asm volatile("cp.async.bulk.tensor.4d.global.shared::cta.bulk_group [%0, {%2, %3, %4, %5}], [%1];"
            :: "l"((uint64_t)map), "r"(SmemAddr(smem)), "r"(c0), "r"(c1), "r"(c2), "r"(c3) : "memory");
    }
    __device__ __forceinline__ void StoreCommit() { asm volatile("cp.async.bulk.commit_group;" ::: "memory"); }
    __device__ __forceinline__ void StoreWaitRead() { asm volatile("cp.async.bulk.wait_group.read 0;" ::: "memory"); }
    __device__ __forceinline__ void StoreWaitAll() { asm volatile("cp.async.bulk.wait_group 0;" ::: "memory"); }
#endif
}
}
```

Measured before the change: 321.8.

## Fold spatial neighbor search into temporal classify and sort into spatial classify

Removes the standalone spatial-search and sort kernels. The neighbor search moves into the temporal classify kernel as a shared device helper, and the sort's per-class ranking and thread-map write move into the spatial classify kernel, which now processes 2x2 pixels per thread over 32x32 tiles. This cuts kernel launches and repeated G-buffer and reservoir reads. In exchange the classify kernels carry more work per thread and use more registers. The neighbor map is now computed once before the spatial passes instead of once per pass.

After: 331.0 (median of 6 runs). 1.03x the previous value.

```diff
diff --git a/zetaray_b200/csrc/rpt.cu b/zetaray_b200/csrc/rpt.cu
--- a/zetaray_b200/csrc/rpt.cu
+++ b/zetaray_b200/csrc/rpt.cu
@@ -275,191 +275,6 @@
                 finalImg[idx] = f4(li.x, li.y, li.z, 0.0f);
         }
     }
-
-    __global__ void __launch_bounds__(256) k_spatial_search(FrameView f, RptParams prm, uint16_t* __restrict__ neighbor)
-    {
-        const zr_frame_constants& fc = f.fc;
-        const uint32_t x = blockIdx.x * 32 + (threadIdx.x & 31);
-        const uint32_t y = prm.rowBegin + blockIdx.y * 8 + (threadIdx.x >> 5);
-        if (x >= f.W || y >= f.H || y >= prm.rowEnd) return;
-        const size_t idx = (size_t)y * f.W + x;
-        const uint4 c = ld128(&f.core[idx]);
-        const GFlags flags = DecodeFlags(c.w & 0xff);
-        if (flags.invalid || flags.emissive) return;
-        const float roughness = (float)((c.w >> 8) & 0xff) / 255.0f;
-        const float viewDepth = asfloat(c.x);
-        const float2 renderDimF = f2((float)f.W, (float)f.H);
-        const float2 jitter = f2(fc.CurrCameraJitter[0], fc.CurrCameraJitter[1]);
-        const float3 pos = Math::WorldPosFromScreenSpace(f2((float)x, (float)y), renderDimF, viewDepth, fc.TanHalfFOV,
-            fc.AspectRatio, fc.CurrViewInv, jitter);
-        const float3 normal = Math::DecodeUnitVector(Math::DecodeUNorm2(c.y));
-        const uint3 h = RNG::PCG3d(make_uint3(x, y, fc.FrameNum));
-        RNG rng = RNG::Init(h.x, h.y, fc.FrameNum);
-        const float u0 = rng.Uniform();
-        const uint32_t offset = rng.UniformUint();
-        const float theta = u0 * TWO_PI;
-        float sinTheta, cosTheta;
-        zr_sincosf(theta, &sinTheta, &cosTheta);
-        int foundX = 0xffff, foundY = 0xffff;
-        int sxs[3], sys[3];
-        bool inside[3];
-        uint4 cand[3];
-#pragma unroll
-        for (uint32_t i = 0; i < 3; i++)
-        {
-            const uint32_t si = (offset + i) & 511;
-            const float2 sampleUV = __ldg(reinterpret_cast<const float2*>(c_disk512) + si);
-            float2 rotated = f2(dot(sampleUV, f2(cosTheta, -sinTheta)), dot(sampleUV, f2(sinTheta, cosTheta)));
-            rotated = rotated * 15.0f;
-            sxs[i] = (int)rintf((float)x + rotated.x); sys[i] = (int)rintf((float)y + rotated.y);
-            inside[i] = !(sxs[i] < 0 || sys[i] < 0 || sxs[i] >= (int)f.W || sys[i] >= (int)f.H) && !(sxs[i] == (int)x && sys[i] == (int)y);
-            cand[i] = inside[i] ? ld128(&f.core[(size_t)sys[i] * f.W + sxs[i]]) : make_uint4(0, 0, 0, 0);
-        }
-#pragma unroll
-        for (uint32_t i = 0; i < 3; i++)
-        {
-            if (foundX != 0xffff || !inside[i]) continue;
-            const int sxp = sxs[i], syp = sys[i];
-            const uint4 sc4 = cand[i];
-            const GFlags sf = DecodeFlags(sc4.w & 0xff);
-            if (sf.invalid || sf.emissive) continue;
-            if (flags.metallic != sf.metallic) continue;
-            if (flags.transmissive != sf.transmissive) continue;
-            const float sampleRoughness = (float)((sc4.w >> 8) & 0xff) / 255.0f;
-            if (fabsf(sampleRoughness - roughness) > 0.05f) continue;
-            const float3 samplePos = Math::WorldPosFromScreenSpace(f2((float)sxp, (float)syp), renderDimF, asfloat(sc4.x),
-                fc.TanHalfFOV, fc.AspectRatio, fc.CurrViewInv, jitter);
-            const float3 sampleNormal = Math::DecodeUnitVector(Math::DecodeUNorm2(sc4.y));
-            if (!(fabsf(dot(normal, samplePos - pos)) <= 0.01f * viewDepth)) continue;
-            if (dot(sampleNormal, normal) < 0.9f) continue;
-            foundX = sxp; foundY = syp;
-        }
-        uint32_t mx, my;
-        if (foundX == 0xffff) { mx = 0xff; my = 0xff; }
-        else { mx = (uint32_t)(foundX - (int)x + 32); my = (uint32_t)(foundY - (int)y + 32); }
-        neighbor[idx] = (uint16_t)((mx & 0xff) | ((my & 0xff) << 8));
-    }
-
-    __global__ void __launch_bounds__(256) k_sort(FrameView f, int mode, uint32_t spatialFlag, const zr_rpt_reservoir* __restrict__ resCurr,
-        const zr_rpt_reservoir* __restrict__ resPrev, const uint16_t* __restrict__ neighbor, uint16_t* __restrict__ threadMap,
-        uint32_t dispX, uint32_t dispY, uint32_t tileRow0)
-    {
-        enum { SUCCESS = 0, INVALID_PIXEL = 1, NOT_FOUND = 2, EMPTY = 4 };
-        __shared__ unsigned long long s_warp[8];
-        const uint32_t Gx = blockIdx.x, Gy = blockIdx.y + tileRow0, Gidx = threadIdx.x;
-        const uint32_t GTx = Gidx & 15, GTy = Gidx >> 4;
-        const bool againstEdge = (Gx == dispX - 1) || (Gy == dispY - 1);
-        const bool lastGroup = (Gx == dispX - 1) && (Gy == dispY - 1);
-        int dxs[4], dys[4], cls[4];
-        uint32_t result[4];
-#pragma unroll
-        for (int i = 0; i < 4; i++)
-        {
-            const int gtx = (int)GTx * 2 + (i & 1), gty = (int)GTy * 2 + (i >> 1);
-            const int dx = (int)(Gx * 32) + gtx, dy = (int)(Gy * 32) + gty;
-            dxs[i] = dx; dys[i] = dy;
-            int nx = 0, ny = 0;
-            uint32_t err = SUCCESS;
-            if ((uint32_t)dx >= f.W || (uint32_t)dy >= f.H)
-                err = INVALID_PIXEL;
-            else
-            {
-                const GFlags flags = FlagsAt(f.core, f.W, dx, dy);
-                if (flags.invalid || flags.emissive)
-                    err = INVALID_PIXEL;
-                else if (mode == 1)
-                {
-                    if (!PrevPixel(f, dx, dy, nx, ny)) err = NOT_FOUND;
-                }
-                else if (mode == 3)
-                {
-                    if (!NeighborOf(f, neighbor, dx, dy, nx, ny)) err = NOT_FOUND;
-                }
-            }
-            bool skip = err != SUCCESS;
-            uint32_t k = Reconnection::EMPTY;
-            if (err == SUCCESS)
-            {
-                const zr_rpt_reservoir* src = (mode == 1) ? resPrev : resCurr;
-                const int sx = (mode == 1 || mode == 3) ? nx : dx, sy = (mode == 1 || mode == 3) ? ny : dy;
-                const uint32_t kk = __ldg(&src[(size_t)sy * f.W + sx].meta) & 0xf;
-                k = kk == Reconnection::EMPTY ? kk : kk + 2;
-            }
-            uint32_t res = err;
-            if (k == Reconnection::EMPTY) { res |= EMPTY; skip = true; }
-            bool edge = false;
-            if (skip && againstEdge && ((uint32_t)dx < f.W) && ((uint32_t)dy < f.H))
-            {
-                res = SUCCESS; skip = false; edge = true;
-            }
-            int c = 4;
-            if (!skip)
-            {
-                if (k == 2) c = 0;
-                else if (k == 3) c = 1;
-                else if (k == 4) c = 2;
-                else c = 3;
-                (void)edge;
-            }
-            cls[i] = c;
-            result[i] = res;
-        }
-        auto writeOutput = [&](int dx, int dy, int mgx, int mgy, uint32_t res)
-        {
-            if ((Gx == dispX - 1) && (Gy != dispY - 1)) { const int t = mgx; mgx = mgy; mgy = t; }
-            const int mx = (int)(Gx * 32) + mgx, my = (int)(Gy * 32) + mgy;
-            uint32_t error;
-            if (mode == 1) error = res & (spatialFlag ? (INVALID_PIXEL | NOT_FOUND) : INVALID_PIXEL);
-            else if (mode == 3) error = res & INVALID_PIXEL;
-            else error = res & (INVALID_PIXEL | EMPTY);
-            if ((uint32_t)mx < f.W && (uint32_t)my < f.H)
-            {
-                const uint32_t ux = (uint32_t)(dx - mx + 31), uy = (uint32_t)(dy - my + 31);
-                threadMap[(size_t)my * f.W + mx] = (uint16_t)(ux | (uy << 7) | ((error > 0 ? 1u : 0u) << 15));
-            }
-        };
-        if (lastGroup)
-        {
-#pragma unroll
-            for (int i = 0; i < 4; i++)
-                writeOutput(dxs[i], dys[i], (int)GTx * 2 + (i & 1), (int)GTy * 2 + (i >> 1), result[i]);
-            return;
-        }
-        unsigned long long mine = 0;
-#pragma unroll
-        for (int i = 0; i < 4; i++) mine += 1ull << (11 * cls[i]);
-        unsigned long long incl = mine;
-        const uint32_t lane = Gidx & 31, warp = Gidx >> 5;
-#pragma unroll
-        for (int off = 1; off < 32; off <<= 1)
-        {
-            const unsigned long long n = __shfl_up_sync(0xffffffffu, incl, off);
-            if (lane >= (uint32_t)off) incl += n;
-        }
-        if (lane == 31) s_warp[warp] = incl;
-        __syncthreads();
-        unsigned long long warpOff = 0, total = 0;
-        for (uint32_t w = 0; w < 8; w++)
-        {
-            const unsigned long long v = s_warp[w];
-            if (w < warp) warpOff += v;
-            total += v;
-        }
-        const unsigned long long excl = warpOff + incl - mine;
-        uint32_t base[5];
-        uint32_t acc = 0;
-#pragma unroll
-        for (int c = 0; c < 5; c++) { base[c] = acc; acc += (uint32_t)((total >> (11 * c)) & 0x7ff); }
-        uint32_t within[5] = { 0, 0, 0, 0, 0 };
-#pragma unroll
-        for (int i = 0; i < 4; i++)
-        {
-            const int c = cls[i];
-            const uint32_t rank = base[c] + (uint32_t)((excl >> (11 * c)) & 0x7ff) + within[c];
-            within[c]++;
-            writeOutput(dxs[i], dys[i], (int)(rank & 31), (int)(rank >> 5), result[i]);
-        }
-    }
 }
 }
 
@@ -480,7 +295,7 @@
     int currTemporalIdx = 0;
     bool isTemporalReservoirValid = false;
     bool resetTemporalTextures = true;
-    bool patternLoaded = false;
+    const float2* d_disk512 = nullptr;
     zr::LightingStrip strip{ "zr_indirect_pass" };
     zr_indirect_params params = Defaults();
 
@@ -529,12 +344,14 @@
 
     zr_status LoadPattern()
     {
-        if (patternLoaded) return ZR_OK;
+        if (d_disk512) return ZR_OK;
         float pat[1024];
         zr_status st = zr::read_asset("zr_indirect_pass", "disk512.bin", pat, sizeof(pat));
         if (st != ZR_OK) return st;
         ZR_CUDA(cudaMemcpyToSymbol(zr::c_disk512, pat, 4096));
-        patternLoaded = true;
+        void* p = nullptr;
+        ZR_CUDA(cudaGetSymbolAddress(&p, zr::c_disk512));
+        d_disk512 = static_cast<const float2*>(p);
         return ZR_OK;
     }
 
@@ -563,7 +380,6 @@
         prm.costMap = strip.d_costMap;
         st = strip.Schedule(width, height, 16, 8, ZR_PT_THREADS / 128);
         if (st != ZR_OK) return st;
-        const uint32_t rows = prm.rowEnd - prm.rowBegin;
 
         int cur = currTemporalIdx;
         const uint32_t dispX = (width + 15) / 16, dispY = (height + 7) / 8;
@@ -574,7 +390,8 @@
         ZR_LAUNCH_CHECK();
         if (doTemporal)
         {
-            st = sz.queued.RunTemporal(shiftStreams, in->scene->dev, f, prm, sz.d_res[cur], sz.d_res[1 - cur], sz.d_target, sz.d_final, plain, stream);
+            st = sz.queued.RunTemporal(shiftStreams, in->scene->dev, f, prm, sz.d_res[cur], sz.d_res[1 - cur], sz.d_target, sz.d_final,
+                doSpatial ? sz.d_neighbor : nullptr, d_disk512, plain, stream);
             if (st != ZR_OK) return st;
         }
         strip.Exchange(sz.d_res[cur], width, height, 64u, stream);
@@ -582,20 +399,9 @@
         {
             for (uint32_t pass = 0; pass < params.num_spatial_passes; pass++)
             {
-                ZR_PROF("k_spatial_search", stream);
-                k_spatial_search<<<dim3((width + 31) / 32, (rows + 7) / 8), 256, 0, stream>>>(f, prm, sz.d_neighbor);
-                ZR_LAUNCH_CHECK();
                 zr_rpt_reservoir* rin = sz.d_res[cur];
                 zr_rpt_reservoir* rout = sz.d_res[1 - cur];
                 cur = 1 - cur;
-                if (params.sort_spatial)
-                {
-                    const uint32_t sx = (width + 31) / 32, sy = (height + 31) / 32;
-                    ZR_PROF("k_sort", stream);
-                    const uint32_t ty0 = prm.rowBegin / 32, ty1 = (prm.rowEnd + 31) / 32;
-                    k_sort<<<dim3(sx, ty1 - ty0), 256, 0, stream>>>(f, 3, 1u, rin, nullptr, sz.d_neighbor, sz.d_threadMap, sx, sy, ty0);
-                    ZR_LAUNCH_CHECK();
-                }
                 st = sz.queued.Run(shiftStreams, in->scene->dev, f, prm, rin, rout, sz.d_target, sz.d_final, sz.d_neighbor, sz.d_threadMap, plain, stream);
                 if (st != ZR_OK) return st;
                 strip.Exchange(rout, width, height, 64u, stream);
diff --git a/zetaray_b200/csrc/rpt_spatial.cu b/zetaray_b200/csrc/rpt_spatial.cu
--- a/zetaray_b200/csrc/rpt_spatial.cu
+++ b/zetaray_b200/csrc/rpt_spatial.cu
@@ -9,29 +9,131 @@
     using namespace RPT;
 
     __global__ void __launch_bounds__(256) k_spatial_classify(FrameView f, RptParams prm, const zr_rpt_reservoir* __restrict__ resIn,
-        const uint16_t* __restrict__ neighbor, uint32_t* __restrict__ queue, uint32_t* __restrict__ counters, uint32_t capacity)
-    {
+        const uint16_t* __restrict__ neighbor, uint16_t* __restrict__ threadMap, uint32_t* __restrict__ queue, uint32_t* __restrict__ counters,
+        uint32_t capacity, uint32_t tileRow0)
+    {
+        enum { SUCCESS = 0, INVALID_PIXEL = 1, NOT_FOUND = 2, EMPTY = 4 };
         __shared__ uint32_t s_count[SpatialQueued::NUM_CLASSES], s_base[SpatialQueued::NUM_CLASSES];
-        const uint32_t x = blockIdx.x * 32 + (threadIdx.x & 31);
-        const uint32_t y = prm.rowBegin + blockIdx.y * 8 + (threadIdx.x >> 5);
+        __shared__ unsigned long long s_warp[8];
+        const uint32_t dispX = (f.W + 31) / 32, dispY = (f.H + 31) / 32;
+        const uint32_t Gx = blockIdx.x, Gy = blockIdx.y + tileRow0, Gidx = threadIdx.x;
+        const uint32_t GTx = Gidx & 15, GTy = Gidx >> 4;
         if (threadIdx.x < SpatialQueued::NUM_CLASSES) s_count[threadIdx.x] = 0;
         __syncthreads();
-        uint32_t cls[2] = { NO_ITEM, NO_ITEM };
-        if (x < f.W && y < f.H && y < prm.rowEnd)
-        {
-            const GFlags flags = FlagsAt(f.core, f.W, (int)x, (int)y);
+        const bool againstEdge = (Gx == dispX - 1) || (Gy == dispY - 1);
+        const bool lastGroup = (Gx == dispX - 1) && (Gy == dispY - 1);
+        int dxs[4], dys[4], sortCls[4];
+        uint32_t result[4];
+        uint32_t cls[8], item[8];
+#pragma unroll
+        for (int i = 0; i < 4; i++)
+        {
+            const int dx = (int)(Gx * 32 + GTx * 2) + (i & 1), dy = (int)(Gy * 32 + GTy * 2) + (i >> 1);
+            dxs[i] = dx; dys[i] = dy;
+            cls[2 * i] = cls[2 * i + 1] = NO_ITEM;
+            item[2 * i] = (uint32_t)dx | ((uint32_t)dy << 16);
+            item[2 * i + 1] = item[2 * i] | (1u << 31);
             int nx = 0, ny = 0;
-            if (!(flags.invalid || flags.emissive) && NeighborOf(f, neighbor, (int)x, (int)y, nx, ny))
-            {
-                const uint4 q0 = ld128(&resIn[(size_t)y * f.W + x]);
+            uint32_t err = SUCCESS, k = Reconnection::EMPTY;
+            if ((uint32_t)dx >= f.W || (uint32_t)dy >= f.H)
+                err = INVALID_PIXEL;
+            else
+            {
+                const GFlags flags = FlagsAt(f.core, f.W, dx, dy);
+                if (flags.invalid || flags.emissive)
+                    err = INVALID_PIXEL;
+                else if (!NeighborOf(f, neighbor, dx, dy, nx, ny))
+                    err = NOT_FOUND;
+            }
+            if (err == SUCCESS)
+            {
                 const uint4 qn = ld128(&resIn[(size_t)ny * f.W + nx]);
-                const bool selfEmpty = (q0.x & 0xf) == Reconnection::EMPTY, nEmpty = (qn.x & 0xf) == Reconnection::EMPTY;
-                const uint32_t M_n = (qn.x >> 4) & 0xf;
-                if (asfloat(q0.y) != 0 && !selfEmpty && M_n > 0) cls[0] = ShiftClass(q0.x);
-                if (!nEmpty) cls[1] = ShiftClass(qn.x);
-            }
-        }
-        const uint32_t item[2] = { x | (y << 16), x | (y << 16) | (1u << 31) };
+                const uint32_t kk = qn.x & 0xf;
+                k = kk == Reconnection::EMPTY ? kk : kk + 2;
+                if ((uint32_t)dy >= prm.rowBegin && (uint32_t)dy < prm.rowEnd)
+                {
+                    const uint4 q0 = ld128(&resIn[(size_t)dy * f.W + dx]);
+                    const bool selfEmpty = (q0.x & 0xf) == Reconnection::EMPTY, nEmpty = kk == Reconnection::EMPTY;
+                    const uint32_t M_n = (qn.x >> 4) & 0xf;
+                    if (asfloat(q0.y) != 0 && !selfEmpty && M_n > 0) cls[2 * i] = ShiftClass(q0.x);
+                    if (!nEmpty) cls[2 * i + 1] = ShiftClass(qn.x);
+                }
+            }
+            bool skip = err != SUCCESS;
+            uint32_t res = err;
+            if (k == Reconnection::EMPTY) { res |= EMPTY; skip = true; }
+            if (skip && againstEdge && ((uint32_t)dx < f.W) && ((uint32_t)dy < f.H))
+            {
+                res = SUCCESS; skip = false;
+            }
+            int c = 4;
+            if (!skip)
+            {
+                if (k == 2) c = 0;
+                else if (k == 3) c = 1;
+                else if (k == 4) c = 2;
+                else c = 3;
+            }
+            sortCls[i] = c;
+            result[i] = res;
+        }
+        if (prm.sortSpatial)
+        {
+            auto writeOutput = [&](int dx, int dy, int mgx, int mgy, uint32_t res)
+            {
+                if ((Gx == dispX - 1) && (Gy != dispY - 1)) { const int t = mgx; mgx = mgy; mgy = t; }
+                const int mx = (int)(Gx * 32) + mgx, my = (int)(Gy * 32) + mgy;
+                const uint32_t error = res & INVALID_PIXEL;
+                if ((uint32_t)mx < f.W && (uint32_t)my < f.H)
+                {
+                    const uint32_t ux = (uint32_t)(dx - mx + 31), uy = (uint32_t)(dy - my + 31);
+                    threadMap[(size_t)my * f.W + mx] = (uint16_t)(ux | (uy << 7) | ((error > 0 ? 1u : 0u) << 15));
+                }
+            };
+            if (lastGroup)
+            {
+#pragma unroll
+                for (int i = 0; i < 4; i++)
+                    writeOutput(dxs[i], dys[i], (int)GTx * 2 + (i & 1), (int)GTy * 2 + (i >> 1), result[i]);
+            }
+            else
+            {
+                unsigned long long mine = 0;
+#pragma unroll
+                for (int i = 0; i < 4; i++) mine += 1ull << (11 * sortCls[i]);
+                unsigned long long incl = mine;
+                const uint32_t lane = Gidx & 31, warp = Gidx >> 5;
+#pragma unroll
+                for (int off = 1; off < 32; off <<= 1)
+                {
+                    const unsigned long long n = __shfl_up_sync(0xffffffffu, incl, off);
+                    if (lane >= (uint32_t)off) incl += n;
+                }
+                if (lane == 31) s_warp[warp] = incl;
+                __syncthreads();
+                unsigned long long warpOff = 0, total = 0;
+                for (uint32_t w = 0; w < 8; w++)
+                {
+                    const unsigned long long v = s_warp[w];
+                    if (w < warp) warpOff += v;
+                    total += v;
+                }
+                const unsigned long long excl = warpOff + incl - mine;
+                uint32_t base[5];
+                uint32_t acc = 0;
+#pragma unroll
+                for (int c = 0; c < 5; c++) { base[c] = acc; acc += (uint32_t)((total >> (11 * c)) & 0x7ff); }
+                uint32_t within[5] = { 0, 0, 0, 0, 0 };
+#pragma unroll
+                for (int i = 0; i < 4; i++)
+                {
+                    const int c = sortCls[i];
+                    const uint32_t rank = base[c] + (uint32_t)((excl >> (11 * c)) & 0x7ff) + within[c];
+                    within[c]++;
+                    writeOutput(dxs[i], dys[i], (int)(rank & 31), (int)(rank >> 5), result[i]);
+                }
+            }
+        }
         AppendItems(cls, item, queue, counters, capacity, s_count, s_base);
     }
 
@@ -42,8 +144,12 @@
         float sum[2][1024];
         uint8_t cls[1024];
         uint8_t visited[1024];
+        uint4 nrec[2][1024];
+        uint4 shStc[1024];
+        float2 shCts[1024];
         unsigned long long bar[2];
     };
+    static_assert(sizeof(MergeSmem) <= 227 * 1024, "k_spatial_merge: MergeSmem exceeds the shared memory of a block");
 
     __global__ void __launch_bounds__(1024, 1) k_spatial_merge(const CUtensorMap* __restrict__ pMapIn, FrameView f, RptParams prm,
         const zr_rpt_reservoir* __restrict__ resIn, zr_rpt_reservoir* __restrict__ resOut, const float4* __restrict__ target,
@@ -92,8 +198,27 @@
             if (sx < f.W && sy < f.H)
                 pfMap = prm.sortSpatial ? __ldg(&threadMap[(size_t)sy * f.W + sx]) : (31u | (31u << 7));
         };
+        auto gather = [&](uint32_t tile)
+        {
+            const GFlags flags = DecodeFlags(pfFlags);
+            const uint32_t ox = pfNb & 0xff, oy = pfNb >> 8;
+            if (!(flags.invalid || flags.emissive) && ox != 0xff)
+            {
+                const int x = (int)((tile % tilesX) * 32 + lane), y = (int)((tileRow0 + tile / tilesX) * 32 + warp);
+                const int nx = (int)ox - 32 + x, ny = (int)oy - 32 + y;
+                const uint4* nrec = reinterpret_cast<const uint4*>(&resIn[(size_t)ny * f.W + nx]);
+                const uint4* sp = reinterpret_cast<const uint4*>(&shiftRes[(size_t)y * f.W + x]);
+                tma::Copy16(&sm.nrec[0][t], &nrec[0]);
+                tma::Copy16(&sm.nrec[1][t], &nrec[1]);
+                tma::Copy16(&sm.shStc[t], &sp[0]);
+                tma::Copy8(&sm.shCts[t], &sp[1]);
+            }
+        };
         if (blockIdx.x < numTiles)
+        {
             prefetch(blockIdx.x);
+            gather(blockIdx.x);
+        }
 
         uint32_t it = 0;
         for (uint32_t tile = blockIdx.x; tile < numTiles; tile += gridDim.x, it++)
@@ -117,36 +242,31 @@
             bool hasN = false;
             const float4 tg = pfTg;
             const uint32_t mapEnc = pfMap;
-            uint4 sh0 = make_uint4(0, 0, 0, 0);
-            float2 sh1 = f2(0, 0);
-            uint4 n0 = make_uint4(Reconnection::EMPTY, 0, 0, 0), n1 = make_uint4(0, 0, 0, 0);
             if (act)
             {
                 const uint32_t ox = pfNb & 0xff, oy = pfNb >> 8;
                 hasN = ox != 0xff;
                 nx = (int)ox - 32 + x; ny = (int)oy - 32 + y;
                 if (hasN)
-                {
-                    const uint4* nrec = reinterpret_cast<const uint4*>(&resIn[(size_t)ny * f.W + nx]);
-                    n0 = __ldg(&nrec[0]); n1 = __ldg(&nrec[1]);
-                    asm volatile("prefetch.global.L1 [%0];" :: "l"(nrec + 2));
-                    const uint4* sp = reinterpret_cast<const uint4*>(&shiftRes[idx]);
-                    sh0 = __ldg(&sp[0]);
-                    sh1 = __ldg(reinterpret_cast<const float2*>(&sp[1]));
-                }
-            }
-            if (tile + gridDim.x < numTiles)
+                    asm volatile("prefetch.global.L1 [%0];" :: "l"(reinterpret_cast<const uint4*>(&resIn[(size_t)ny * f.W + nx]) + 2));
+            }
+            const bool more = tile + gridDim.x < numTiles;
+            if (more)
                 prefetch(tile + gridDim.x);
             sm.visited[t] = 0;
+            tma::CopyWaitAll();
             tma::MbarWait(reinterpret_cast<uint64_t*>(&sm.bar[stage]), parity);
 
-            zr_rpt_reservoir rec;
+            auto ownRecord = [&]()
             {
                 const uint4* line = &sm.rec[stage][t & ~1u][0];
                 const uint32_t c0 = (t & 1u) * 4u, sw = swizzled ? ((t >> 1) & 7u) : 0u;
                 uint4 v[4] = { line[(c0 + 0) ^ sw], line[(c0 + 1) ^ sw], line[(c0 + 2) ^ sw], line[(c0 + 3) ^ sw] };
-                memcpy(&rec, v, 64);
-            }
+                zr_rpt_reservoir r;
+                memcpy(&r, v, 64);
+                return r;
+            };
+            const zr_rpt_reservoir rec = ownRecord();
             Reservoir r_curr = Reservoir::Load_NonReconnection(rec);
             r_curr.target = f3(tg.x, tg.y, tg.z);
             const float wsum0 = act ? r_curr.w_sum : 0.0f;
@@ -161,10 +281,14 @@
             else if (act)
             {
                 memset(&recN, 0, sizeof(recN));
-                memcpy(&recN, &n0, 16); memcpy(reinterpret_cast<unsigned char*>(&recN) + 16, &n1, 16);
+                {
+                    const uint4 n0 = sm.nrec[0][t], n1 = sm.nrec[1][t];
+                    memcpy(&recN, &n0, 16); memcpy(reinterpret_cast<unsigned char*>(&recN) + 16, &n1, 16);
+                }
                 r_spatial = Reservoir::Load_NonReconnection(recN);
                 if ((r_curr.w_sum != 0) && !r_curr.rc.Empty() && (r_spatial.M > 0))
                 {
+                    const float2 sh1 = sm.shCts[t];
                     const float target_spatial = sh1.x;
                     if (target_spatial > 0)
                     {
@@ -186,6 +310,7 @@
                     M_max = r_spatial.rc.x_k_in_motion ? (M_max < 4 ? M_max : 4) : M_max;
                     r_spatial.rc.x_k_in_motion = false;
                     const float nJ = (r_spatial.rc.IsCase3() && r_spatial.rc.lobe_k_min_1 == BSDF::ALL) ? 1.0f : asfloat(recN.jacobian_or_seed_nee);
+                    const uint4 sh0 = sm.shStc[t];
                     const float3 shTarget = f3(asfloat(sh0.x), asfloat(sh0.y), asfloat(sh0.z));
                     const float shJ = fabsf(asfloat(sh0.w));
                     surfKMin1Tr = (sh0.w >> 31) != 0;
@@ -217,6 +342,8 @@
                     r_curr.M = M_new;
                 }
             }
+            if (more)
+                gather(tile + gridDim.x);
             sm.val[0][t] = wsum0;
             sm.val[1][t] = act ? r_curr.w_sum : 0.0f;
             sm.cls[t] = (uint8_t)cls;
@@ -252,7 +379,7 @@
                 {
                     if (prm.boilingSuppression) SuppressOutlier(avgEx0, r_curr);
                     WriteOutputColor(fc, finalImg, idx, r_curr.target * r_curr.W);
-                    CopyToNextFrame(rec, &resOut[idx], r_curr, M_max);
+                    CopyToNextFrame(ownRecord(), &resOut[idx], r_curr, M_max);
                 }
                 else if (cls == 2)
                 {
@@ -260,7 +387,7 @@
                     const float targetLum = Math::Luminance(r_curr.target);
                     r_curr.W = targetLum > 0 ? r_curr.w_sum / targetLum : 0;
                     r_curr.M = M_new;
-                    CopyToNextFrame(rec, &resOut[idx], r_curr, M_max);
+                    CopyToNextFrame(ownRecord(), &resOut[idx], r_curr, M_max);
                     WriteOutputColor(fc, finalImg, idx, r_curr.target * r_curr.W);
                 }
                 else
@@ -275,7 +402,7 @@
                         StoreRecord(&resOut[idx], out);
                     }
                     else
-                        CopyToNextFrame(rec, &resOut[idx], r_curr, M_max);
+                        CopyToNextFrame(ownRecord(), &resOut[idx], r_curr, M_max);
                     WriteOutputColor(fc, finalImg, idx, r_curr.target * r_curr.W);
                 }
             }
@@ -348,15 +475,17 @@
 }
 
 zr_status SpatialQueued::Run(const ShiftStreams& ss, const SceneDev& sc, const FrameView& f, const RptParams& prm, const zr_rpt_reservoir* resIn,
-    zr_rpt_reservoir* resOut, const float4* target, float4* finalImg, const uint16_t* neighbor, const uint16_t* threadMap, bool plain, cudaStream_t stream)
+    zr_rpt_reservoir* resOut, const float4* target, float4* finalImg, const uint16_t* neighbor, uint16_t* threadMap, bool plain, cudaStream_t stream)
 {
     const int plane = resIn == mapBase[0] ? 0 : (resIn == mapBase[1] ? 1 : -1);
     if (plane < 0) { set_error("zr_indirect_pass: spatial input is not one of the pass's reservoir planes"); return ZR_ERR_INVALID_ARG; }
-    const uint32_t rows = prm.rowEnd - prm.rowBegin;
+    const uint32_t tilesX = (width + 31) / 32;
+    const uint32_t tileRow0 = prm.rowBegin / 32, tileRow1 = (prm.rowEnd + 31) / 32;
     ZR_CUDA(cudaMemsetAsync(d_counters, 0, 16 * sizeof(uint32_t), stream));
     {
         ZR_PROF("k_spatial_classify", stream);
-        k_spatial_classify<<<dim3((width + 31) / 32, (rows + 7) / 8), 256, 0, stream>>>(f, prm, resIn, neighbor, d_queue, d_counters, (uint32_t)capacity);
+        k_spatial_classify<<<dim3(tilesX, tileRow1 - tileRow0), 256, 0, stream>>>(f, prm, resIn, neighbor, threadMap, d_queue, d_counters,
+            (uint32_t)capacity, tileRow0);
         ZR_LAUNCH_CHECK();
     }
     {
@@ -368,8 +497,6 @@
         if (e != cudaSuccess) return zr::cuda_fail(e, "k_shift launch");
     }
     {
-        const uint32_t tilesX = (width + 31) / 32;
-        const uint32_t tileRow0 = prm.rowBegin / 32, tileRow1 = (prm.rowEnd + 31) / 32;
         const uint32_t numTiles = tilesX * (tileRow1 - tileRow0);
         const uint32_t grid = numTiles < (uint32_t)ss.numSMs ? numTiles : (uint32_t)ss.numSMs;
         ZR_PROF("k_spatial_merge", stream);
diff --git a/zetaray_b200/csrc/rpt_temporal.cu b/zetaray_b200/csrc/rpt_temporal.cu
--- a/zetaray_b200/csrc/rpt_temporal.cu
+++ b/zetaray_b200/csrc/rpt_temporal.cu
@@ -10,7 +10,7 @@
 
     __global__ void __launch_bounds__(256) k_temporal_classify(SceneDev sc, FrameView f, RptParams prm, const zr_rpt_reservoir* __restrict__ resCurr,
         const zr_rpt_reservoir* __restrict__ resPrev, uint8_t* __restrict__ tflags, uint32_t* __restrict__ queue, uint32_t* __restrict__ counters,
-        uint32_t capacity)
+        uint32_t capacity, uint16_t* __restrict__ neighbor, const float2* __restrict__ disk)
     {
         __shared__ uint32_t s_count[SpatialQueued::NUM_CLASSES], s_base[SpatialQueued::NUM_CLASSES];
         const int x = (int)(blockIdx.x * 32 + (threadIdx.x & 31));
@@ -22,8 +22,11 @@
         if (x < (int)f.W && y < (int)f.H && y < (int)prm.rowEnd)
         {
             const size_t idx = (size_t)y * f.W + x;
-            const GFlags flags = DecodeFlags(ld128(&f.core[idx]).w & 0xff);
+            const uint4 c = ld128(&f.core[idx]);
+            const GFlags flags = DecodeFlags(c.w & 0xff);
             bool ok = !(flags.invalid || flags.emissive), okReplay = false;
+            if (ok && neighbor)
+                neighbor[idx] = SpatialSearch(f, disk, (uint32_t)x, (uint32_t)y, c);
             int ppx = 0, ppy = 0;
             if (ok)
             {
@@ -176,14 +179,15 @@
 }
 
 zr_status SpatialQueued::RunTemporal(const ShiftStreams& ss, const SceneDev& sc, const FrameView& f, const RptParams& prm, zr_rpt_reservoir* resCurr,
-    const zr_rpt_reservoir* resPrev, float4* target, float4* finalImg, bool plain, cudaStream_t stream)
+    const zr_rpt_reservoir* resPrev, float4* target, float4* finalImg, uint16_t* neighbor, const float2* disk, bool plain, cudaStream_t stream)
 {
     const uint32_t rows = prm.rowEnd - prm.rowBegin;
     const dim3 grid((width + 31) / 32, (rows + 7) / 8);
     ZR_CUDA(cudaMemsetAsync(d_counters, 0, 16 * sizeof(uint32_t), stream));
     {
         ZR_PROF("k_temporal_classify", stream);
-        k_temporal_classify<<<grid, 256, 0, stream>>>(sc, f, prm, resCurr, resPrev, d_flags, d_queue, d_counters, (uint32_t)capacity);
+        k_temporal_classify<<<grid, 256, 0, stream>>>(sc, f, prm, resCurr, resPrev, d_flags, d_queue, d_counters, (uint32_t)capacity,
+            neighbor, disk);
         ZR_LAUNCH_CHECK();
     }
     {
diff --git a/zetaray_b200/csrc/zr_rpt_io.cuh b/zetaray_b200/csrc/zr_rpt_io.cuh
--- a/zetaray_b200/csrc/zr_rpt_io.cuh
+++ b/zetaray_b200/csrc/zr_rpt_io.cuh
@@ -40,6 +40,64 @@
         if (ox == 0xff) return false;
         nx = ox - 32 + x; ny = oy - 32 + y;
         return true;
+    }
+
+    ZR_D uint16_t SpatialSearch(const FrameView& f, const float2* __restrict__ disk, uint32_t x, uint32_t y, uint4 c)
+    {
+        const zr_frame_constants& fc = f.fc;
+        const GFlags flags = DecodeFlags(c.w & 0xff);
+        const float roughness = (float)((c.w >> 8) & 0xff) / 255.0f;
+        const float viewDepth = asfloat(c.x);
+        const float2 renderDimF = f2((float)f.W, (float)f.H);
+        const float2 jitter = f2(fc.CurrCameraJitter[0], fc.CurrCameraJitter[1]);
+        const float3 pos = Math::WorldPosFromScreenSpace(f2((float)x, (float)y), renderDimF, viewDepth, fc.TanHalfFOV,
+            fc.AspectRatio, fc.CurrViewInv, jitter);
+        const float3 normal = Math::DecodeUnitVector(Math::DecodeUNorm2(c.y));
+        const uint3 h = RNG::PCG3d(make_uint3(x, y, fc.FrameNum));
+        RNG rng = RNG::Init(h.x, h.y, fc.FrameNum);
+        const float u0 = rng.Uniform();
+        const uint32_t offset = rng.UniformUint();
+        const float theta = u0 * TWO_PI;
+        float sinTheta, cosTheta;
+        zr_sincosf(theta, &sinTheta, &cosTheta);
+        int foundX = 0xffff, foundY = 0xffff;
+        int sxs[3], sys[3];
+        bool inside[3];
+        uint4 cand[3];
+#pragma unroll
+        for (uint32_t i = 0; i < 3; i++)
+        {
+            const uint32_t si = (offset + i) & 511;
+            const float2 sampleUV = __ldg(disk + si);
+            float2 rotated = f2(dot(sampleUV, f2(cosTheta, -sinTheta)), dot(sampleUV, f2(sinTheta, cosTheta)));
+            rotated = rotated * 15.0f;
+            sxs[i] = (int)rintf((float)x + rotated.x); sys[i] = (int)rintf((float)y + rotated.y);
+            inside[i] = !(sxs[i] < 0 || sys[i] < 0 || sxs[i] >= (int)f.W || sys[i] >= (int)f.H) && !(sxs[i] == (int)x && sys[i] == (int)y);
+            cand[i] = inside[i] ? ld128(&f.core[(size_t)sys[i] * f.W + sxs[i]]) : make_uint4(0, 0, 0, 0);
+        }
+#pragma unroll
+        for (uint32_t i = 0; i < 3; i++)
+        {
+            if (foundX != 0xffff || !inside[i]) continue;
+            const int sxp = sxs[i], syp = sys[i];
+            const uint4 sc4 = cand[i];
+            const GFlags sf = DecodeFlags(sc4.w & 0xff);
+            if (sf.invalid || sf.emissive) continue;
+            if (flags.metallic != sf.metallic) continue;
+            if (flags.transmissive != sf.transmissive) continue;
+            const float sampleRoughness = (float)((sc4.w >> 8) & 0xff) / 255.0f;
+            if (fabsf(sampleRoughness - roughness) > 0.05f) continue;
+            const float3 samplePos = Math::WorldPosFromScreenSpace(f2((float)sxp, (float)syp), renderDimF, asfloat(sc4.x),
+                fc.TanHalfFOV, fc.AspectRatio, fc.CurrViewInv, jitter);
+            const float3 sampleNormal = Math::DecodeUnitVector(Math::DecodeUNorm2(sc4.y));
+            if (!(fabsf(dot(normal, samplePos - pos)) <= 0.01f * viewDepth)) continue;
+            if (dot(sampleNormal, normal) < 0.9f) continue;
+            foundX = sxp; foundY = syp;
+        }
+        uint32_t mx, my;
+        if (foundX == 0xffff) { mx = 0xff; my = 0xff; }
+        else { mx = (uint32_t)(foundX - (int)x + 32); my = (uint32_t)(foundY - (int)y + 32); }
+        return (uint16_t)((mx & 0xff) | ((my & 0xff) << 8));
     }
 
     ZR_D void SuppressOutlier(float waveAvgExclusive, Reservoir& r)
diff --git a/zetaray_b200/csrc/zr_rpt_shift.cuh b/zetaray_b200/csrc/zr_rpt_shift.cuh
--- a/zetaray_b200/csrc/zr_rpt_shift.cuh
+++ b/zetaray_b200/csrc/zr_rpt_shift.cuh
@@ -164,29 +164,37 @@
         return ZR_OK;
     }
 
-    ZR_D void AppendItems(const uint32_t cls[2], const uint32_t item[2], uint32_t* __restrict__ queue, uint32_t* __restrict__ counters,
+    template<int N>
+    ZR_D void AppendItems(const uint32_t (&cls)[N], const uint32_t (&item)[N], uint32_t* __restrict__ queue, uint32_t* __restrict__ counters,
         uint32_t capacity, uint32_t* s_count, uint32_t* s_base)
     {
         const uint32_t lane = threadIdx.x & 31;
-        uint32_t offs[2] = { 0, 0 };
+        uint32_t offs[N];
         const uint32_t lt = (1u << lane) - 1;
+#pragma unroll
+        for (int d = 0; d < N; d++) offs[d] = 0;
 #pragma unroll
         for (uint32_t c = 0; c < SpatialQueued::NUM_CLASSES; c++)
         {
-            const uint32_t m0 = __ballot_sync(0xffffffffu, cls[0] == c), m1 = __ballot_sync(0xffffffffu, cls[1] == c);
-            const uint32_t n0 = __popc(m0), n = n0 + __popc(m1);
+            uint32_t m[N], n = 0;
+#pragma unroll
+            for (int d = 0; d < N; d++) { m[d] = __ballot_sync(0xffffffffu, cls[d] == c); n += __popc(m[d]); }
             uint32_t base = 0;
             if (n && lane == 0) base = atomicAdd(&s_count[c], n);
             base = __shfl_sync(0xffffffffu, base, 0);
-            if (cls[0] == c) offs[0] = base + __popc(m0 & lt);
-            if (cls[1] == c) offs[1] = base + n0 + __popc(m1 & lt);
+#pragma unroll
+            for (int d = 0; d < N; d++)
+            {
+                if (cls[d] == c) offs[d] = base + __popc(m[d] & lt);
+                base += __popc(m[d]);
+            }
         }
         __syncthreads();
         if (threadIdx.x < SpatialQueued::NUM_CLASSES)
             s_base[threadIdx.x] = s_count[threadIdx.x] ? atomicAdd(&counters[threadIdx.x], s_count[threadIdx.x]) : 0;
         __syncthreads();
 #pragma unroll
-        for (uint32_t d = 0; d < 2; d++)
+        for (int d = 0; d < N; d++)
             if (cls[d] != NO_ITEM)
                 queue[(size_t)cls[d] * capacity + s_base[cls[d]] + offs[d]] = item[d];
     }
diff --git a/zetaray_b200/csrc/zr_rpt_spatial.h b/zetaray_b200/csrc/zr_rpt_spatial.h
--- a/zetaray_b200/csrc/zr_rpt_spatial.h
+++ b/zetaray_b200/csrc/zr_rpt_spatial.h
@@ -44,9 +44,10 @@
 
     zr_status Build(uint32_t w, uint32_t h, const zr_rpt_reservoir* res0, const zr_rpt_reservoir* res1);
     zr_status Run(const ShiftStreams& ss, const SceneDev& sc, const FrameView& f, const RptParams& prm, const zr_rpt_reservoir* resIn,
-        zr_rpt_reservoir* resOut, const float4* target, float4* finalImg, const uint16_t* neighbor, const uint16_t* threadMap, bool plain,
+        zr_rpt_reservoir* resOut, const float4* target, float4* finalImg, const uint16_t* neighbor, uint16_t* threadMap, bool plain,
         cudaStream_t stream);
     zr_status RunTemporal(const ShiftStreams& ss, const SceneDev& sc, const FrameView& f, const RptParams& prm, zr_rpt_reservoir* resCurr,
-        const zr_rpt_reservoir* resPrev, float4* target, float4* finalImg, bool plain, cudaStream_t stream);
+        const zr_rpt_reservoir* resPrev, float4* target, float4* finalImg, uint16_t* neighbor, const float2* disk, bool plain,
+        cudaStream_t stream);
 };
 }
diff --git a/zetaray_b200/csrc/zr_tma.cuh b/zetaray_b200/csrc/zr_tma.cuh
--- a/zetaray_b200/csrc/zr_tma.cuh
+++ b/zetaray_b200/csrc/zr_tma.cuh
@@ -113,6 +113,16 @@
     __device__ __forceinline__ void StoreCommit() { asm volatile("cp.async.bulk.commit_group;" ::: "memory"); }
     __device__ __forceinline__ void StoreWaitRead() { asm volatile("cp.async.bulk.wait_group.read 0;" ::: "memory"); }
     __device__ __forceinline__ void StoreWaitAll() { asm volatile("cp.async.bulk.wait_group 0;" ::: "memory"); }
+
+    __device__ __forceinline__ void Copy16(void* smem, const void* gmem)
+    {
+        asm volatile("cp.async.cg.shared.global [%0], [%1], 16;" :: "r"(SmemAddr(smem)), "l"(gmem) : "memory");
+    }
+    __device__ __forceinline__ void Copy8(void* smem, const void* gmem)
+    {
+        asm volatile("cp.async.ca.shared.global [%0], [%1], 8;" :: "r"(SmemAddr(smem)), "l"(gmem) : "memory");
+    }
+    __device__ __forceinline__ void CopyWaitAll() { asm volatile("cp.async.wait_all;" ::: "memory"); }
 #endif
 }
 }
```
